# cl-volume-renderer/cl-volume-renderer

Measured on AMD Instinct MI355X. Metric: msamples_per_sec, higher is better.
Workload: dtype f32

## Files before the change

cl_volume_renderer_amd/csrc/bounce_device.hpp:

```cpp
#pragma once
#include "render_device.hpp"

namespace clvr {

__device__ __forceinline__ VolumePacked make_volume(const RenderArgs &a) {
  return VolumePacked{a.grec, a.stepb, a.volume_lin, a.sdf_lin, a.X, a.Y, a.Z, a.NBX, a.NBY};
}

__device__ __forceinline__ uint32_t udivmod24(uint32_t n, uint32_t d, uint32_t &rem) {
  uint32_t q = (uint32_t)((float)n * __builtin_amdgcn_rcpf((float)d));
  uint32_t qd;
  asm("v_mul_u32_u24 %0, %1, %2" : "=v"(qd) : "v"(q), "v"(d));
  int32_t r = (int32_t)(n - qd);
  if (r < 0) { q -= 1u; r += (int32_t)d; }
  if (r >= (int32_t)d) { q += 1u; r -= (int32_t)d; }
  rem = (uint32_t)r;
  return q;
}

__device__ __forceinline__ unsigned prefix_count(unsigned long long mask) {
  return __builtin_amdgcn_mbcnt_hi((unsigned)(mask >> 32), __builtin_amdgcn_mbcnt_lo((unsigned)mask, 0u));
}
__device__ __forceinline__ unsigned lane_id() { return prefix_count(~0ull); }

enum : int { ST_IDLE = 0, ST_MARCH = 1, ST_CERT = 2, ST_EVENT = 8 };
enum : int { EV_START = 3,
             EV_HIT_COLOR_PENDING = 4,
             EV_CHECK = 5 };
constexpr int kCertNever = 255;

template <int MODE>
__device__ __forceinline__ void finish_item(const RenderArgs &a, int64_t entry, uint32_t hit, uint32_t gx, uint32_t gy,
                                            uint32_t bv_r, uint32_t bv_g, uint32_t bv_b) {
  const uint32_t cr = (bv_r / 2u) & 0xFFFFu, cg = (bv_g / 2u) & 0xFFFFu, cb = (bv_b / 2u) & 0xFFFFu;
  if (MODE == CLWH_ACCUM_VOXEL_CACHE && a.grants == nullptr) {
    cache_add(a.cache, entry, cr, cg, cb, 0u);
  } else {
    const unsigned long long packed = (unsigned long long)cr | ((unsigned long long)cg << 16) |
                                      ((unsigned long long)cb << 32) | (1ull << 48);
    atomicAdd(a.delta + hit, packed);
  }
  if (a.contrib_out) {
    uint32_t *q = a.contrib_out + ((size_t)gy * (size_t)a.launch_w + gx) * 4;
    q[0] = cr; q[1] = cg; q[2] = cb; q[3] = 1u;
  }
}

constexpr int kFixupDwords = 32;

__device__ __forceinline__ bool certify_exit(const RenderArgs &a, f3 p, f3 d, int budget, int &away) {
  const unsigned cx = min((unsigned)(int)p.x >> a.macro_shift, (unsigned)a.MNX - 1u), cy = min((unsigned)(int)p.y >> a.macro_shift, (unsigned)a.MNY - 1u),
                 cz = min((unsigned)(int)p.z >> a.macro_shift, (unsigned)a.MNZ - 1u);
  const unsigned octant = (d.x < 0.0f ? 1u : 0u) | (d.y < 0.0f ? 2u : 0u) | (d.z < 0.0f ? 4u : 0u);
  const int entry = a.macro[(((cz * (unsigned)a.MNY + cy) * (unsigned)a.MNX + cx) << 3) | octant];
  const bool refused = (entry & (int)kCertRefused) != 0;
  const int box_min = refused ? 0 : entry;
  away = refused ? ((entry & 0x7F) - 1) << a.macro_shift : 0;
  const float dmin = fminf(fminf(fabsf(d.x), fabsf(d.y)), fabsf(d.z));
  const float dsum = d.x + d.y + d.z;
  const float T = (float)((budget - 5) * box_min);
  const float fx = d.x < 0.0f ? p.x : (float)a.X - p.x, fy = d.y < 0.0f ? p.y : (float)a.Y - p.y, fz = d.z < 0.0f ? p.z : (float)a.Z - p.z;
  const bool leaves = T * fabsf(d.x) >= fx || T * fabsf(d.y) >= fy || T * fabsf(d.z) >= fz;
  return box_min != 0 && budget > 5 && leaves && dmin >= 0.0009765625f && dsum == dsum;
}
__device__ __forceinline__ bool start_certificate(uint32_t mask, f3 d, float dmin_needed) {
  const unsigned octant = (d.x < 0.0f ? 1u : 0u) | (d.y < 0.0f ? 2u : 0u) | (d.z < 0.0f ? 4u : 0u);
  const float dmin = fminf(fminf(fabsf(d.x), fabsf(d.y)), fabsf(d.z));
  const float dsum = d.x + d.y + d.z;
  return ((mask >> octant) & 1u) != 0u && dmin >= dmin_needed && dsum == dsum;
}
__device__ __forceinline__ f3 hull_direction(unsigned k) {
  static_assert(kHullGrid == 64, "cell centres are odd multiples of 1/64");
  const float u = (float)(2 * (int)(k & 63u) - 63) * 0.015625f, v = (float)(2 * (int)((k >> 6) & 63u) - 63) * 0.015625f;
  const float z = (1.0f - fabsf(u)) - fabsf(v);
  const float x = z >= 0.0f ? u : copysignf(1.0f - fabsf(v), u), y = z >= 0.0f ? v : copysignf(1.0f - fabsf(u), v);
  const float r = __builtin_amdgcn_rsqf((x * x + y * y) + z * z);
  return f3{x * r, y * r, z * r};
}
__device__ __forceinline__ bool hull_certificate(uint32_t code, f3 d, float delta0) {
  const f3 n = hull_direction(code - 1u);
  const float dmin = fminf(fminf(fabsf(d.x), fabsf(d.y)), fabsf(d.z));
  const float dsum = d.x + d.y + d.z;
  return code != 0u && dot3(d, n) >= delta0 && dmin >= 0.0009765625f && dsum == dsum;
}
__device__ __forceinline__ bool certify_exit(const RenderArgs &a, f3 p, f3 d, int budget) {
  int away;
  return certify_exit(a, p, d, budget, away);
}

template <int SMALL>
__device__ __forceinline__ void index_tables_to_lds(VolumePacked &vol, const RenderArgs &a, int threads) {
  extern __shared__ uint32_t lds_parts[];
  if (SMALL == 2) {
    vol.parts = lds_parts;
    vol.parts_y0 = a.X;
    vol.parts_z0 = a.X + a.Y;
    for (int k = (int)threadIdx.x; k < a.X + a.Y + a.Z; k += threads)
      lds_parts[k] = k < a.X ? vol.part_x<1>((unsigned)k) : (k < a.X + a.Y ? vol.part_y<1>((unsigned)(k - a.X)) : vol.part_z<1>((unsigned)(k - a.X - a.Y)));
  }
}
__device__ __forceinline__ unsigned home_queue_of(const RenderArgs &a, unsigned waves_per_block) {
  unsigned home_queue = (unsigned)__builtin_amdgcn_s_getreg((3 << 11) | 20) & 7u;
  if (a.unit_affinity == 1) home_queue = (blockIdx.x * waves_per_block + (threadIdx.x >> 6)) & 7u;
  if (a.unit_affinity == 2) home_queue = 0u;
  return home_queue;
}

#ifdef CLVR_BOUNCE_STATS
constexpr bool kBounceStats = true;
constexpr bool kStartCertVerify = (CLVR_BOUNCE_STATS + 0) != 2;
#else
constexpr bool kBounceStats = false;
constexpr bool kStartCertVerify = false;
#endif
template <bool ON> struct BounceStatsT;
template <> struct BounceStatsT<false> {
  __device__ void step(int) {}
  __device__ void cert_begin(int, int) {}
  __device__ void cert_end(int, int) {}
  __device__ void closing_half(int) {}
  __device__ void event_phase(int) {}
  __device__ void refill(uint32_t) {}
  __device__ void fresh_items(int, int) {}
  __device__ void swap_point() {}
  __device__ void start_cert(bool, bool) {}
  __device__ void hull_cert(bool, bool, bool) {}
  __device__ void march_end(uint32_t *, int) {}
  template <bool TWO_RAYS> __device__ void flush(uint32_t *) {}
};
template <> struct BounceStatsT<true> {
  uint32_t step_iters = 0, step_lanes = 0, event_phases = 0, event_lanes = 0, refills = 0, refill_lanes = 0;
  uint32_t ev_kind[4] = {0, 0, 0, 0};
  uint32_t cert_phases = 0, cert_lanes = 0, cert_granted = 0;
  uint32_t step_idle = 0;
  uint32_t swaps = 0;
  uint32_t closing = 0, marching_before = 0;
  __device__ __forceinline__ void step(int st) {
    step_iters += 1; step_lanes += (uint32_t)__popcll(__ballot(st == ST_MARCH));
    step_idle += (uint32_t)__popcll(__ballot(st == ST_IDLE));
  }
  __device__ __forceinline__ void cert_begin(int st, int n_cert) {
    cert_phases += 1; cert_lanes += (uint32_t)n_cert;
    marching_before = (uint32_t)__popcll(__ballot(st == ST_MARCH));
  }
  __device__ __forceinline__ void cert_end(int st, int n_cert) { cert_granted += (uint32_t)(n_cert - (__popcll(__ballot(st == ST_MARCH)) - (int)marching_before)); }
  __device__ __forceinline__ void closing_half(int st) {
    closing = (uint32_t)__popcll(__ballot(st >= ST_EVENT));
    event_lanes += closing;
    ev_kind[1] += (uint32_t)__popcll(__ballot(st == ST_EVENT + EV_EXIT || st == ST_EVENT + EV_CHECK));
    ev_kind[2] += (uint32_t)__popcll(__ballot(st == ST_EVENT + EV_HIT || st == ST_EVENT + EV_HIT_COLOR_PENDING));
    ev_kind[3] += (uint32_t)__popcll(__ballot(st == ST_EVENT + EV_NONE));
  }
  __device__ __forceinline__ void event_phase(int st) {
    if (__ballot(st >= ST_EVENT) != 0ull) { event_phases += 1; event_lanes += (uint32_t)__popcll(__ballot(st >= ST_EVENT)); }
  }
  __device__ __forceinline__ void refill(uint32_t count) { refills += 1; refill_lanes += count; }
  __device__ __forceinline__ void fresh_items(int st, int o) {
    const uint32_t n_fresh = (uint32_t)__popcll(__ballot(st == ST_EVENT + EV_START && o == 1));
    ev_kind[0] += n_fresh; event_lanes += n_fresh;
    if (closing + n_fresh != 0u) event_phases += 1;
  }
  __device__ __forceinline__ void swap_point() { swaps += 1; }
  uint32_t start_tried = 0, start_granted = 0;
  bool start_open = false;
  __device__ __forceinline__ void start_cert(bool tried, bool granted) {
    start_tried += (uint32_t)__popcll(__ballot(tried)); start_granted += (uint32_t)__popcll(__ballot(granted));
    start_open = start_open || granted;
  }
  uint32_t hull_tried = 0, hull_granted = 0, hull_both = 0;
  bool hull_open = false;
  __device__ __forceinline__ void hull_cert(bool tried, bool granted, bool both) {
    hull_tried += (uint32_t)__popcll(__ballot(tried)); hull_granted += (uint32_t)__popcll(__ballot(granted));
    hull_both += (uint32_t)__popcll(__ballot(both));
    hull_open = hull_open || granted;
  }
  __device__ __forceinline__ void march_end(uint32_t *counters, int ev) {
    if (start_open && ev != EV_EXIT) atomicAdd(&counters[CTR_START_WRONG], 1u);
    if (hull_open && ev != EV_EXIT) atomicAdd(&counters[CTR_HULL_WRONG], 1u);
    start_open = false;
    hull_open = false;
  }
  template <bool TWO_RAYS> __device__ __forceinline__ void flush(uint32_t *counters) {
    atomicAdd(&counters[CTR_STEP_ITERS], step_iters); atomicAdd(&counters[CTR_STEP_LANES], step_lanes);
    atomicAdd(&counters[CTR_EVENT_PHASES], event_phases); atomicAdd(&counters[CTR_EVENT_LANES], event_lanes);
    atomicAdd(&counters[CTR_REFILLS], refills); atomicAdd(&counters[CTR_REFILL_LANES], refill_lanes);
    if (TWO_RAYS) { atomicAdd(&counters[CTR_SWAPS], swaps); return; }
    for (int k = 0; k < 4; ++k) atomicAdd(&counters[CTR_EV_KIND + k], ev_kind[k]);
    atomicAdd(&counters[CTR_CERT_PHASES], cert_phases); atomicAdd(&counters[CTR_CERT_LANES], cert_lanes);
    atomicAdd(&counters[CTR_CERT_GRANTED], cert_granted); atomicAdd(&counters[CTR_STEP_IDLE], step_idle);
    atomicAdd(&counters[CTR_START_TRIED], start_tried); atomicAdd(&counters[CTR_START_GRANTED], start_granted);
    atomicAdd(&counters[CTR_HULL_TRIED], hull_tried); atomicAdd(&counters[CTR_HULL_GRANTED], hull_granted); atomicAdd(&counters[CTR_HULL_BOTH], hull_both);
  }
};
using BounceStats = BounceStatsT<kBounceStats>;

}
```

cl_volume_renderer_amd/csrc/clwh_context.hip:

```cpp
#include <algorithm>
#include <cstdio>
#include <cstdlib>
#include <cstring>
#include <mutex>
#include <new>

#include "clwh_host.hpp"

using namespace clvr;

static thread_local int g_last_hip_error = 0;
void clvr::note_hip_error(hipError_t e) { g_last_hip_error = (int)e; }

static std::atomic<uint64_t> g_content_version{0};
static std::mutex g_cells_mutex;
static std::map<const void *, std::weak_ptr<VersionCell>> g_version_cells;
void clwh_touch(clwh_mem *m) { m->cell->v.store(++g_content_version, std::memory_order_relaxed); }

static std::shared_ptr<VersionCell> version_cell_of(const void *dptr) {
  std::lock_guard<std::mutex> lock(g_cells_mutex);
  auto it = g_version_cells.find(dptr);
  if (it != g_version_cells.end())
    if (auto live = it->second.lock()) return live;
  auto cell = std::make_shared<VersionCell>();
  g_version_cells[dptr] = cell;
  if (g_version_cells.size() > 4096) {
    for (auto i = g_version_cells.begin(); i != g_version_cells.end();)
      i = i->second.expired() ? g_version_cells.erase(i) : std::next(i);
  }
  return cell;
}

static size_t elem_size(int kind) {
  switch (kind) {
    case CLWH_ELEM_S8: case CLWH_ELEM_U8: return 1;
    case CLWH_ELEM_S16: case CLWH_ELEM_U16: return 2;
    case CLWH_ELEM_S32: case CLWH_ELEM_U32: case CLWH_ELEM_F32: return 4;
    default: return 0;
  }
}


void clvr::tf_to_dev(const clwh_tf &tf, TfDev &d) {
  std::memset(&d, 0, sizeof d);
  d.n = tf.n;
  for (int k = 0; k < tf.n; ++k) {
    const clwh_tf_rule &r = tf.rules[k];
    TfRuleDev &o = d.rules[k];
    o.v_lo = r.v_lo; o.v_hi = r.v_hi; o.g_lo = r.g_lo; o.g_hi = r.g_hi;
    o.flags = (r.use_gradient ? TF_USE_GRADIENT : 0u) | (r.writes_color ? TF_WRITES_COLOR : 0u) |
              (r.terminal ? TF_TERMINAL : 0u);
    o.color = ((uint32_t)r.color[0] & 255u) | (((uint32_t)r.color[1] & 255u) << 8) |
              (((uint32_t)r.color[2] & 255u) << 16) | (((uint32_t)r.color[3] & 255u) << 24);
    if (r.use_gradient) d.uses_gradient = 1;
  }
  for (int k = 0; k < tf.n && !d.uses_gradient; ++k) {
    const clwh_tf_rule &r = tf.rules[k];
    if (r.v_lo <= 0 && 0 <= r.v_hi) { d.border_class = k + 1; break; }
    if (r.terminal) break;
  }
}

int clvr::jit_for_source(clwh_ctx *ctx, const char *source, std::shared_ptr<JitTf> &out) {
  auto it = ctx->classes.cache.find(source);
  if (it != ctx->classes.cache.end()) {
    out = it->second;
    return CLWH_OK;
  }
  auto j = std::make_shared<JitTf>();
  j->source = source;
  std::string log;
  const int rc = tf_jit_compile(source, j->code, log);
  if (rc != CLWH_OK) {
    if (!log.empty()) std::fprintf(stderr, "clwhip: transfer-function source is neither in the rule grammar nor compilable:\n%s\n", log.c_str());
    return rc;
  }
  ctx->classes.cache[source] = j;
  out = j;
  return CLWH_OK;
}

int clvr::ensure_classes(clwh_ctx *ctx, const std::shared_ptr<JitTf> &jit, const clwh_mem *volume, TfDev &tf_out, const uint8_t **cls_out) {
  TfClasses &c = ctx->classes;
  if (c.cls.ptr && c.vol == volume->dptr && c.vol_ver == volume->version() && c.source == jit->source) {
    tf_out = c.tf;
    *cls_out = c.cls.as<uint8_t>();
    return CLWH_OK;
  }
  if (!jit->module) {
    HIP_TRY(hipModuleLoadData(&jit->module, jit->code.data()));
    HIP_TRY(hipModuleGetFunction(&jit->classify, jit->module, "clvr_tf_classify"));
  }
  const size_t voxels = volume->dims[0] * volume->dims[1] * volume->dims[2];
  CLWH_TRY(c.cls.reserve(ctx->stream, voxels));
  constexpr int kColors = CLWH_TF_MAX_RULES;
  CLWH_TRY(c.palette.reserve(ctx->stream, (kColors + 2) * sizeof(unsigned long long)));
  unsigned long long *palette = c.palette.as<unsigned long long>();
  HIP_TRY(hipMemsetAsync(palette, 0xFF, kColors * sizeof(unsigned long long), ctx->stream));
  HIP_TRY(hipMemsetAsync(palette + kColors, 0, 2 * sizeof(unsigned long long), ctx->stream));
  const void *vol = volume->dptr;
  int X = (int)volume->dims[0], Y = (int)volume->dims[1], Z = (int)volume->dims[2], max_colors = kColors;
  unsigned char *cls = c.cls.as<unsigned char>();
  int *error = reinterpret_cast<int *>(palette + kColors);
  int *border = reinterpret_cast<int *>(palette + kColors + 1);
  void *args[] = {&vol, &X, &Y, &Z, &cls, &palette, &max_colors, &error, &border};
  const size_t blocks = std::min<size_t>((voxels + 255u) / 256u, (size_t)1u << 23);
  HIP_TRY(hipModuleLaunchKernel(jit->classify, (unsigned)blocks, 1, 1, 256, 1, 1, 0, ctx->stream, args, nullptr));
  unsigned long long host[kColors + 2];
  HIP_TRY(hipMemcpyAsync(host, palette, sizeof host, hipMemcpyDeviceToHost, ctx->stream));
  HIP_TRY(hipStreamSynchronize(ctx->stream));
  c.vol = nullptr;
  if ((int)(host[kColors] & 0xFFFFFFFFull) != 0) return CLWH_ERR_TF_UNSUPPORTED;
  TfDev t;
  std::memset(&t, 0, sizeof t);
  t.opaque = 1;
  for (int k = 0; k < kColors && host[k] != ~0ull; ++k) {
    t.rules[k].flags = (host[k] >> 32) & 1ull ? TF_WRITES_COLOR : 0u;
    t.rules[k].color = (uint32_t)(host[k] & 0xFFFFFFFFull);
    t.n = k + 1;
  }
  t.border_class = (int32_t)(host[kColors + 1] & 0xFFull);
  c.tf = t;
  c.vol = volume->dptr;
  c.vol_ver = volume->version();
  c.source = jit->source;
  tf_out = t;
  *cls_out = cls;
  return CLWH_OK;
}


Tuning clvr::tuning_from_environment() {
  Tuning t;
  auto clamped = [](const char *e, int lo, int hi) { return std::max(lo, std::min(hi, std::atoi(e))); };
  if (const char *e = std::getenv("CLWH_TUNE_STEP")) t.step_min_lanes = clamped(e, 0, 64);
  if (const char *e = std::getenv("CLWH_TUNE_REFILL")) t.refill_min_lanes = clamped(e, 0, 64);
  if (const char *e = std::getenv("CLWH_TUNE_LITERAL_GRADIENT")) t.literal_gradient = std::atoi(e) != 0;
  if (const char *e = std::getenv("CLWH_TUNE_AFFINITY")) t.unit_affinity = std::atoi(e);
  if (const char *e = std::getenv("CLWH_TUNE_QUEUES")) t.unit_queues = clamped(e, 1, 8);
  if (const char *e = std::getenv("CLWH_TUNE_GROUP")) t.unit_group = std::max(1, std::atoi(e));
  if (const char *e = std::getenv("CLWH_TUNE_CHUNK_BLOCK_LOG2")) t.unit_block_log2 = clamped(e, 0, 8);
  if (const char *e = std::getenv("CLWH_TUNE_BLOCKS")) t.bounce_max_blocks = (uint32_t)std::max(1, std::atoi(e));
  if (const char *e = std::getenv("CLWH_TUNE_MACRO_SHIFT")) t.macro_shift = std::atoi(e);
  if (const char *e = std::getenv("CLWH_TUNE_LONG_LAUNCH")) t.force_long_launch = std::atoi(e) != 0;
  if (const char *e = std::getenv("CLWH_TUNE_BOUNCE_RAYS")) t.bounce_rays = std::atoi(e) == 2 ? 2 : 1;
  if (const char *e = std::getenv("CLWH_TUNE_SDF")) t.sdf_front = std::strcmp(e, "front") == 0;
  if (const char *e = std::getenv("CLWH_TUNE_DIST_LINES")) t.dist_lines = std::strcmp(e, "scan") == 0 ? 1 : std::strcmp(e, "search") == 0 ? 2 : 0;
  if (const char *e = std::getenv("CLWH_TUNE_LABEL_STATS")) t.label_stats = std::strcmp(e, "item") == 0 ? 1 : std::strcmp(e, "direct") == 0 ? 2 : 0;
  if (const char *e = std::getenv("CLWH_TUNE_SLICE_COARSE")) t.slice_coarse = std::atoi(e) != 0;
  if (const char *e = std::getenv("CLWH_TUNE_SDFBIT_WAVES")) t.sdfbit_waves = std::atoi(e) == 16 ? 16 : 8;
  if (const char *e = std::getenv("CLWH_TUNE_SDFBIT_GRID")) t.sdfbit_grid = std::max(1, std::atoi(e));
  if (const char *e = std::getenv("CLWH_TUNE_SDFBIT_REC")) t.sdfbit_rec_lds = std::strcmp(e, "lds") == 0 ? 1 : 0;
  if (const char *e = std::getenv("CLWH_TUNE_CERT")) t.cert_min_step = clamped(e, 0, 127);
  if (const char *e = std::getenv("CLWH_TUNE_CERT_HINT")) t.cert_hint = std::atoi(e) != 0;
  if (const char *e = std::getenv("CLWH_TUNE_START_CERT")) t.start_cert = std::atoi(e) != 0;
  if (const char *e = std::getenv("CLWH_TUNE_HULL_CERT")) t.hull_cert = std::atoi(e) != 0;
  return t;
}

int clvr::check_device_flags(clwh_ctx *ctx) {
  PassScratch &p = ctx->pass;
  if (!p.fixup_overflow_pending || !p.sticky_flags.ptr) return CLWH_OK;
  uint32_t flag = 0;
  HIP_TRY(hipMemcpyAsync(&flag, p.sticky_flags.ptr, sizeof flag, hipMemcpyDeviceToHost, ctx->stream));
  HIP_TRY(hipStreamSynchronize(ctx->stream));
  p.fixup_overflow_pending = false;
  if (!flag) return CLWH_OK;
  HIP_TRY(hipMemsetAsync(p.sticky_flags.ptr, 0, sizeof(uint32_t), ctx->stream));
  return CLWH_ERR_INTERNAL_OVERFLOW;
}

int clvr::timed_begin(clwh_ctx *ctx, int which, hipEvent_t *end) {
  LaunchTimers &t = ctx->timers;
  if (!t.enabled) return CLWH_OK;
  if (t.used == t.pairs.size()) {
    LaunchTimers::Pair &fresh = t.pairs.emplace_back();
    int rc = fresh.begin.ensure(hipEventDefault);
    if (rc == CLWH_OK) rc = fresh.end.ensure(hipEventDefault);
    if (rc != CLWH_OK) {
      t.pairs.pop_back();
      return rc;
    }
  }
  LaunchTimers::Pair &p = t.pairs[t.used++];
  p.which = which;
  HIP_TRY(hipEventRecord(p.begin.ev, ctx->stream));
  *end = p.end.ev;
  return CLWH_OK;
}

static int order_streams(clwh_ctx *ctx, hipStream_t first, hipStream_t then) {
  HIP_TRY(hipSetDevice(ctx->device));
  CLWH_TRY(ctx->handoff.ensure(hipEventDisableTiming));
  HIP_TRY(hipEventRecord(ctx->handoff.ev, first));
  HIP_TRY(hipStreamWaitEvent(then, ctx->handoff.ev, 0));
  return CLWH_OK;
}

extern "C" {

int clwh_ctx_create_on_stream(int device, void *hip_stream, clwh_ctx **out) {
  if (!out) return CLWH_ERR_INVALID_VALUE;
  *out = nullptr;
  int count = 0;
  hipError_t e = hipGetDeviceCount(&count);
  if (e != hipSuccess || count <= 0) {
    note_hip_error(e);
    return CLWH_ERR_NO_DEVICE;
  }
  if (device < 0 || device >= count) return CLWH_ERR_NO_DEVICE;
  HIP_TRY(hipSetDevice(device));
  clwh_ctx *c = new (std::nothrow) clwh_ctx();
  if (!c) return CLWH_ERR_OUT_OF_MEMORY;
  c->device = device;
  c->stream = (hipStream_t)hip_stream;
  c->own_stream = false;
  c->tune = tuning_from_environment();
  *out = c;
  return CLWH_OK;
}

int clwh_ctx_create(int device, clwh_ctx **out) {
  CLWH_TRY(clwh_ctx_create_on_stream(device, nullptr, out));
  hipStream_t s;
  hipError_t e = hipStreamCreateWithFlags(&s, hipStreamNonBlocking);
  if (e != hipSuccess) {
    note_hip_error(e);
    delete *out;
    *out = nullptr;
    return CLWH_ERR_HIP;
  }
  (*out)->stream = s;
  (*out)->own_stream = true;
  return CLWH_OK;
}

int clwh_ctx_destroy(clwh_ctx *ctx) {
  if (!ctx) return CLWH_ERR_INVALID_VALUE;
  (void)hipSetDevice(ctx->device);
  (void)hipStreamSynchronize(ctx->stream);
  for (auto &kv : ctx->classes.cache)
    if (kv.second->module) (void)hipModuleUnload(kv.second->module);
  ctx->scene.reset();
  const hipStream_t owned = ctx->own_stream ? ctx->stream : nullptr;
  delete ctx;
  if (owned) (void)hipStreamDestroy(owned);
  return CLWH_OK;
}

int clwh_ctx_finish(clwh_ctx *ctx) {
  if (!ctx) return CLWH_ERR_INVALID_VALUE;
  HIP_TRY(hipStreamSynchronize(ctx->stream));
  return check_device_flags(ctx);
}

int clwh_ctx_acquire_from(clwh_ctx *ctx, void *hip_stream) {
  if (!ctx) return CLWH_ERR_INVALID_VALUE;
  return order_streams(ctx, (hipStream_t)hip_stream, ctx->stream);
}

int clwh_ctx_release_to(clwh_ctx *ctx, void *hip_stream) {
  if (!ctx) return CLWH_ERR_INVALID_VALUE;
  return order_streams(ctx, ctx->stream, (hipStream_t)hip_stream);
}

void *clwh_ctx_stream(clwh_ctx *ctx) { return ctx ? (void *)ctx->stream : nullptr; }
int clwh_ctx_device(clwh_ctx *ctx) { return ctx ? ctx->device : -1; }

int clwh_ctx_set_timing(clwh_ctx *ctx, int enabled) {
  if (!ctx) return CLWH_ERR_INVALID_VALUE;
  ctx->timers.enabled = enabled != 0;
  ctx->timers.used = 0;
  return CLWH_OK;
}

int clwh_ctx_timing_read_all(clwh_ctx *ctx, float *ms, int32_t *launches, int32_t n) {
  if (!ctx || !ms || !launches || n <= 0) return CLWH_ERR_INVALID_VALUE;
  for (int k = 0; k < n; ++k) { ms[k] = 0.0f; launches[k] = 0; }
  HIP_TRY(hipSetDevice(ctx->device));
  LaunchTimers &timers = ctx->timers;
  for (size_t i = 0; i < timers.used; ++i) {
    const LaunchTimers::Pair &p = timers.pairs[i];
    HIP_TRY(hipEventSynchronize(p.end.ev));
    float t = 0.0f;
    HIP_TRY(hipEventElapsedTime(&t, p.begin.ev, p.end.ev));
    if (p.which >= 0 && p.which < n) { ms[p.which] += t; launches[p.which] += 1; }
  }
  timers.used = 0;
  return CLWH_OK;
}

int clwh_ctx_timing_read(clwh_ctx *ctx, float *total_ms, int32_t *launches) {
  if (!ctx || !total_ms || !launches) return CLWH_ERR_INVALID_VALUE;
  float ms[CLWH_TIMER_COUNT];
  int32_t n[CLWH_TIMER_COUNT];
  const int rc = clwh_ctx_timing_read_all(ctx, ms, n, CLWH_TIMER_COUNT);
  *total_ms = ms[CLWH_TIMER_BOUNCE];
  *launches = n[CLWH_TIMER_BOUNCE];
  return rc;
}


static int mem_new(clwh_ctx *ctx, void *dptr, size_t bytes, bool owned, clwh_mem **out) {
  clwh_mem *m = new (std::nothrow) clwh_mem();
  if (!m) return CLWH_ERR_OUT_OF_MEMORY;
  m->ctx = ctx;
  m->dptr = dptr;
  m->bytes = bytes;
  m->owned = owned;
// ... 155 lines not shown
```

cl_volume_renderer_amd/csrc/clwh_host.hpp:

```cpp
#pragma once

#include <atomic>
#include <deque>
#include <map>
#include <memory>
#include <string>
#include <vector>

#include "clwh_internal.hpp"

namespace clvr {

void note_hip_error(hipError_t e);
inline int hip_failed(hipError_t e) {
  note_hip_error(e);
  return e == hipErrorOutOfMemory ? CLWH_ERR_OUT_OF_MEMORY : CLWH_ERR_HIP;
}
#define HIP_TRY(expr)                                   \
  do {                                                  \
    hipError_t _e = (expr);                             \
    if (_e != hipSuccess) return clvr::hip_failed(_e);  \
  } while (0)
#define CLWH_TRY(expr)                \
  do {                                \
    int _rc = (expr);                 \
    if (_rc != CLWH_OK) return _rc;   \
  } while (0)

struct NoCopy {
  NoCopy() = default;
  NoCopy(const NoCopy &) = delete;
  NoCopy &operator=(const NoCopy &) = delete;
};

struct DeviceBuffer : NoCopy {
  void *ptr = nullptr;
  size_t bytes = 0;
  ~DeviceBuffer() { if (ptr) (void)hipFree(ptr); }
  template <class T>
  T *as() const { return static_cast<T *>(ptr); }
  void *release() {
    void *p = ptr;
    ptr = nullptr;
    bytes = 0;
    return p;
  }
  int reserve(hipStream_t stream, size_t need, bool *reallocated = nullptr) {
    if (reallocated) *reallocated = bytes < need;
    if (bytes >= need) return CLWH_OK;
    if (ptr) {
      HIP_TRY(hipStreamSynchronize(stream));
      HIP_TRY(hipFree(ptr));
      (void)release();
    }
    HIP_TRY(hipMalloc(&ptr, need));
    bytes = need;
    return CLWH_OK;
  }
};

struct Event : NoCopy {
  hipEvent_t ev = nullptr;
  ~Event() { if (ev) (void)hipEventDestroy(ev); }
  int ensure(unsigned flags) {
    if (!ev) HIP_TRY(hipEventCreateWithFlags(&ev, flags));
    return CLWH_OK;
  }
};

struct PinnedWord : NoCopy {
  uint32_t *ptr = nullptr;
  ~PinnedWord() { if (ptr) (void)hipHostFree(ptr); }
  int ensure() {
    if (!ptr) HIP_TRY(hipHostMalloc((void **)&ptr, 64, hipHostMallocDefault));
    return CLWH_OK;
  }
};

int tf_jit_compile(const char *user_source, std::vector<char> &code, std::string &log);
struct JitTf {
  std::string source;
  std::vector<char> code;
  hipModule_t module = nullptr;
  hipFunction_t classify = nullptr;
};

struct PackedScene {
  int device = 0;
  DeviceBuffer data;
  const void *vol = nullptr, *sdf = nullptr;
  uint64_t vol_ver = 0, sdf_ver = 0;
  TfDev tf{};
  std::string tf_identity;
  int32_t macro_shift = 0;
  bool start_table = false;
  bool hull_table = false;
  int32_t dims[3] = {0, 0, 0};
  uint64_t generation = 0;
  Event ready;
  bool stale = false;
  ~PackedScene();
};

struct VersionCell {
  std::atomic<uint64_t> v{0};
};


struct Tuning {
  int32_t step_min_lanes = 0;
  int32_t refill_min_lanes = 0;
  int32_t macro_shift = 0;
  int32_t bounce_rays = 1;
  int32_t force_long_launch = 0;
  int32_t literal_gradient = 0;
  int32_t unit_block_log2 = 4;
  int32_t unit_group = 1, unit_affinity = 0, unit_queues = 8;
  int32_t cert_hint = 1;
  int32_t start_cert = 1;
  int32_t hull_cert = 1;
  int32_t cert_min_step = -1;
  uint32_t bounce_max_blocks = 2048;
  int32_t sdfbit_waves = 8;
  int32_t sdfbit_grid = 512;
  int32_t sdfbit_rec_lds = 0;
  int32_t sdf_front = 0;
  int32_t dist_lines = 0;
  int32_t label_stats = 0;
  int32_t slice_coarse = 1;
};
Tuning tuning_from_environment();

struct PrimaryHits {
  struct Key {
    float cam_pos[3], cam_dir[3];
    int32_t frame_w, frame_h, launch_w, launch_h, tile_rank, tile_world;
    int64_t cache_entries;
    int32_t mode, shading;
    uint64_t packed_generation;
    const void *env;
    uint64_t env_version;
    int32_t env_w, env_h;
  } key{};
  bool valid = false;
  DeviceBuffer pix_slot, hits;
  DeviceBuffer hull_codes;
  uint32_t n_hits = 0;
  bool n_hits_known = false;
  PinnedWord host_n_hits;
  Event n_hits_event;
  bool n_hits_in_flight = false;
  uint32_t last_known_n_hits = 0;
};

struct PassScratch {
  static constexpr size_t kCounters = CTR_QUEUE_STRIDE * 9;
  DeviceBuffer counters;
  DeviceBuffer fixups, delta;
  DeviceBuffer sticky_flags;
  bool fixup_overflow_pending = false;
};

struct VoxelPlan {
  DeviceBuffer plan;
  DeviceBuffer temp;
  bool valid = false;
  uint32_t n = 0;
};

struct TfClasses {
  std::map<std::string, std::shared_ptr<JitTf>> cache;
  DeviceBuffer cls;
  DeviceBuffer palette;
  const void *vol = nullptr;
  uint64_t vol_ver = 0;
  std::string source;
  TfDev tf{};
};

struct SdfScratch {
  DeviceBuffer counters;
  DeviceBuffer flags;
  DeviceBuffer bits;
#ifdef CLVR_SDFBIT_TIMING
  DeviceBuffer timing;
#endif
};

struct GrowScratch {
  DeviceBuffer admissible, tiles, seeds;
  PinnedWord host;
};

struct LabelScratch {
  DeviceBuffer admissible, keys, temp, counters;
  PinnedWord host;
};

struct DistanceScratch {
  DeviceBuffer map_a, map_b, bits;
};

struct RegionStatsScratch {
  DeviceBuffer result;
};

struct OverlayScratch {
  DeviceBuffer pixel_ids, occupancy;
};

struct ProjectionData {
  DeviceBuffer data;
  bool valid = false;
  const void *vol = nullptr;
  uint64_t vol_ver = 0;
  size_t dims[3] = {0, 0, 0};
  DeviceBuffer dilated;
  bool dilated_valid = false;
  DeviceBuffer mesh_counts, mesh_temp, mesh_points;
  DeviceBuffer lut_prefix;
  bool lut_valid = false;
  const void *lut = nullptr;
  uint64_t lut_ver = 0;
  int32_t lut_len = 0;
};

struct LaunchTimers {
  struct Pair {
    Event begin, end;
    int which = 0;
  };
  bool enabled = false;
  std::deque<Pair> pairs;
  size_t used = 0;
};

}

struct clwh_ctx {
  int device = 0;
  hipStream_t stream = nullptr;
  bool own_stream = false;
  clvr::Event handoff;
  clvr::Tuning tune;
  clvr::PrimaryHits primary;
  clvr::PassScratch pass;
  clvr::VoxelPlan vox;
  clvr::TfClasses classes;
  clvr::SdfScratch sdf;
  clvr::GrowScratch grow;
  clvr::LabelScratch label;
  clvr::DistanceScratch distance;
  clvr::RegionStatsScratch region_stats;
  clvr::OverlayScratch overlay;
  clvr::ProjectionData proj;
  clvr::DeviceBuffer bilateral_weights;
  std::shared_ptr<clvr::PackedScene> scene;
  clvr::LaunchTimers timers;
};

struct clwh_mem {
  clwh_ctx *ctx = nullptr;
  void *dptr = nullptr;
  size_t bytes = 0;
  bool owned = false;
  bool is_image = false;
  size_t dims[3] = {1, 1, 1};
  int channels = 1;
  int elem_kind = CLWH_ELEM_U8;
  int flags = 0;
  std::shared_ptr<clvr::VersionCell> cell;
  uint64_t version() const { return cell ? cell->v.load(std::memory_order_relaxed) : 0; }
};

enum clwh_kernel_id {
  CLWH_K_EMPTY = 0,
  CLWH_K_RENDER,
  CLWH_K_SDF_BASE,
  CLWH_K_SDF_LAYER,
  CLWH_K_BUFFER_RESET,
  CLWH_K_FETCH_STATS,
  CLWH_K_APPLY_CLIP,
  CLWH_K_TF_SORT_VALUES,
  CLWH_K_TF_FLUSH_COLOR_FRAME,
  CLWH_K_BILATERAL_FILTER
};

struct clwh_kernel {
  clwh_ctx *ctx = nullptr;
  int id = CLWH_K_EMPTY;
  clwh_tf tf{};
  bool has_tf = false;
  std::shared_ptr<clvr::JitTf> jit;
};

void clwh_touch(clwh_mem *m);

namespace clvr {

inline void touch(clwh_mem *m) { clwh_touch(m); }

int check_device_flags(clwh_ctx *ctx);

void tf_to_dev(const clwh_tf &tf, TfDev &d);
int jit_for_source(clwh_ctx *ctx, const char *source, std::shared_ptr<JitTf> &out);
int ensure_classes(clwh_ctx *ctx, const std::shared_ptr<JitTf> &jit, const clwh_mem *volume, TfDev &tf_out, const uint8_t **cls_out);
inline int kernel_tf(clwh_kernel *k, const clwh_mem *volume, TfDev &tf_out, const uint8_t **cls_out) {
  if (k->jit) return ensure_classes(k->ctx, k->jit, volume, tf_out, cls_out);
  tf_to_dev(k->tf, tf_out);
// ... 36 lines not shown
```

cl_volume_renderer_amd/csrc/clwh_internal.hpp:

```cpp
#pragma once

#include <hip/hip_runtime.h>
#include <stdint.h>

#include "../../include/clwh.h"

namespace clvr {

struct TfRuleDev {
  int32_t v_lo, v_hi, g_lo, g_hi;
  uint32_t flags;
  uint32_t color;
};
struct TfDev {
  int32_t n;
  int32_t uses_gradient;
  int32_t literal_gradient_taps;
  int32_t opaque;
  int32_t border_class;
  TfRuleDev rules[CLWH_TF_MAX_RULES];
};

enum : uint32_t { TF_USE_GRADIENT = 1u, TF_WRITES_COLOR = 2u, TF_TERMINAL = 4u };

struct HitRec {
  float origin[3];
  float direction[3];
  float normal[3];
  uint32_t color;
  int32_t entry_lo;
  int32_t entry_hi;
  uint32_t xy;
  uint32_t pslot;
  uint32_t start_free;
  uint32_t pad;
};
static_assert(sizeof(HitRec) == 64, "HitRec must be one 64-byte line");

enum : uint32_t { PIX_HIT = 0x80000000u };

constexpr uint32_t kCertMinStep = 2u;
constexpr uint32_t kCertRefused = 0x80u;

enum : uint32_t {
  CTR_HITS = 0, CTR_FIXUPS = 2,
  CTR_STEP_ITERS = 8, CTR_STEP_LANES, CTR_EVENT_PHASES, CTR_EVENT_LANES, CTR_REFILLS, CTR_REFILL_LANES,
  CTR_EV_KIND,
  CTR_CERT_PHASES = CTR_EV_KIND + 4, CTR_CERT_LANES, CTR_CERT_GRANTED,
  CTR_SWAPS, CTR_STEP_IDLE,
  CTR_START_TRIED, CTR_START_GRANTED, CTR_START_WRONG,
  CTR_HULL_TRIED, CTR_HULL_GRANTED, CTR_HULL_BOTH, CTR_HULL_WRONG,
  CTR_STATS_END,
  CTR_QUEUE_STRIDE = 32,
};
struct RenderArgs {
  int32_t X, Y, Z;
  const uint2 *grec;
  const uint8_t *stepb;
  const int16_t *volume_lin;
  const int8_t *sdf_lin;
  const uint8_t *macro;
  int32_t MNX, MNY, MNZ, macro_shift;
  int32_t cert_min_step;
  int32_t cert_min_lanes;
  int32_t cert_hint;
  const uint8_t *start_free;
  float start_cert_dmin;
  const float4 *hull;
  uint32_t *hull_codes;
  float hull_delta0;
  int32_t NBX, NBY;
  const uint32_t *env;
  int32_t env_w, env_h;
  uint32_t *cache;
  int64_t cache_entries;
  uint32_t *frame;
  int32_t frame_w, frame_h;
  int32_t launch_w, launch_h;
  int32_t tiles_x, tiles_y, tiles_per_row;
  int32_t tile_rank, tile_world;
  float cam_pos[3];
  float cam_dir[3];
  int32_t mode;
  float4 *accum;
  unsigned long long *delta;
  const uint32_t *grants;
  uint32_t *pix_slot;
  HitRec *hits;
  uint32_t *counters;
  uint32_t *fixups;
  uint32_t fixup_capacity;
  uint32_t *sticky_flags;
  uint32_t n_hits;
  uint32_t n_hits_estimate;
  int32_t n_hits_on_device;
  int32_t shading;
  int64_t *hit_index_out;
  uint32_t *contrib_out;
  uint32_t num_tile_slots;
  int32_t n_seeds;
  int32_t seeds[CLWH_MAX_SEEDS];
  int32_t step_min_lanes;
  int32_t refill_min_lanes;
  int32_t force_long_launch;
  int32_t bounce_rays;
  uint32_t bounce_max_blocks;
  int32_t unit_group;
  int32_t unit_block_log2;
  int32_t unit_queues;
  int32_t unit_affinity;
  TfDev tf;
};

struct RepackArgs {
  const int16_t *volume;
  const int8_t *sdf;
  int32_t X, Y, Z;
  int32_t NBX, NBY, NBZ;
  uint2 *grec;
  uint8_t *stepb;
  uint32_t *brick_min;
  const uint8_t *cls_in;
  TfDev tf;
};

struct SdfArgs {
  const int16_t *volume;
  int32_t X, Y, Z;
  int8_t *ping;
  int8_t *pong;
  int32_t max_iterations;
  int32_t iteration;
  int32_t *counters;
  int32_t *done;
  int32_t *counter_out;
  const uint8_t *cls_in;
  TfDev tf;
};

hipError_t launch_repack(const RepackArgs &a, hipStream_t s);
inline int macro_cell_shift(int X, int Y, int Z, int forced) {
  if (forced >= 3 && forced <= 8) return forced;
  auto cells = [&](int sh) { return (int64_t)((X >> sh) + 1) * ((Y >> sh) + 1) * ((Z >> sh) + 1); };
  int shift = 4;
  if (cells(4) > 40000) {
    shift = 5;
    while (shift < 8 && cells(shift) > 300000) ++shift;
  }
  return shift;
}
hipError_t launch_macro_table(const uint32_t *brick_min, int NBX, int NBY, int NBZ, uint8_t *macro, int X, int Y, int Z, int shift, hipStream_t s);
hipError_t launch_start_table(const uint8_t *stepb, uint8_t *table, uint32_t *regular, int2 *ends, int X, int Y, int Z, int NBX, int NBY, int NBZ, hipStream_t s);
inline int start_cert_cap(int X, int Y, int Z) {
  const int longest = X > Y ? (X > Z ? X : Z) : (Y > Z ? Y : Z);
  return longest / 2 < 127 ? longest / 2 : 127;
}
inline float start_cert_dmin(int X, int Y, int Z) {
  const double longest = (double)(X > Y ? (X > Z ? X : Z) : (Y > Z ? Y : Z));
  const double reach = 1.7320508075688772 * (longest + 1.0), cap = (double)start_cert_cap(X, Y, Z);
  for (int k = 1; k <= 64; ++k) {
    const double dmin = (double)k / 64.0;
    double t = 0.0;
    for (int step = 0; step < 70 - 5 && t <= reach; ++step) {
      const double m = (double)(long long)(t * dmin) - 2.0;
      const double bound = m > cap ? cap : m;
      t += bound < 1.0 ? 1.0 : bound;
    }
    if (t > reach) return (float)dmin;
  }
  return 2.0f;
}
constexpr int kHullGrid = 64;
constexpr int kHullPlanes = kHullGrid * kHullGrid;
constexpr float kHullSlack = 0.0625f;
constexpr int kHullMaxDim = 2048;
inline float hull_cert_delta0(int X, int Y, int Z) {
  const double longest = (double)(X > Y ? (X > Z ? X : Z) : (Y > Z ? Y : Z));
  const double reach = 1.7320508075688772 * (longest + 1.0), cap = (double)start_cert_cap(X, Y, Z);
  for (int k = 1; k <= 64; ++k) {
    const double delta0 = (double)k / 64.0;
    double t = 0.0;
    for (int step = 0; step < 70 - 5 && t <= reach; ++step) {
      const double m = (double)(long long)(t * delta0 / 1.7320508075688772) - 2.0;
      const double bound = m > cap ? cap : m;
      t += bound < 1.0 ? 1.0 : bound;
    }
    if (t > reach) return (float)delta0;
  }
  return 2.0f;
}
hipError_t launch_hull_table(const int2 *ends, const uint32_t *regular, float4 *hull, int X, int Y, int Z, hipStream_t s);
constexpr uint64_t kStartTableBudget = 2ull << 30;
hipError_t launch_primary(const RenderArgs &a, hipStream_t s);
hipError_t launch_bounce(const RenderArgs &a, hipStream_t s);
inline bool bounce_queues_fit(uint32_t n_hits, int32_t unit_block_log2, int32_t n_seeds) {
  return (uint64_t)(((n_hits + 63u) >> 6) + 8u * (1u << unit_block_log2)) * (uint64_t)n_seeds < (1ull << 24);
}
hipError_t launch_env_fixup(const RenderArgs &a, hipStream_t s);
hipError_t launch_commit(const RenderArgs &a, hipStream_t s);
constexpr int64_t kVoxKeyInvalid = (int64_t)1 << 38;
constexpr int64_t kVoxKeyNone = ((int64_t)1 << 38) + 1;
hipError_t launch_vox_keys(const RenderArgs &a, int64_t *keys, uint32_t *iota, uint32_t n, hipStream_t s);
hipError_t launch_vox_grant(const RenderArgs &a, const int64_t *sorted_keys, const uint32_t *order, uint32_t n, uint32_t *grants, hipStream_t s);
hipError_t launch_commit_voxel(const RenderArgs &a, hipStream_t s);
hipError_t sort_entry_pairs(void *temp, size_t &temp_bytes, const int64_t *keys_in, int64_t *keys_out, const uint32_t *vals_in,
                            uint32_t *vals_out, size_t n, unsigned end_bit, hipStream_t s);
hipError_t launch_resolve(const RenderArgs &a, hipStream_t s);
hipError_t launch_ao(const RenderArgs &a, hipStream_t s);
hipError_t launch_accum_resolve(const RenderArgs &a, const float4 *accum_all, hipStream_t s);
hipError_t launch_accum_resolve_tiles(const RenderArgs &a, const float4 *accum, uint32_t *tiles_out, hipStream_t s);
hipError_t launch_frame_from_tiles(const RenderArgs &a, const uint32_t *tiles_all, hipStream_t s);
struct SdfFrontArgs {
  int8_t *sdf;
  int32_t X, Y, Z;
  int32_t TX, TY, TZ;
  const uint8_t *flags_cur;
  uint8_t *flags_next;
  uint8_t *flags_clear;
  uint8_t *tile_done;
  int32_t iteration;
  int32_t max_iterations;
  int32_t *counters;
};

struct SdfBitArgs {
  int8_t *sdf;
  const uint32_t *ev;
  const uint32_t *r_in;
  uint32_t *r_out;
  uint8_t *state;
  uint8_t *wake;
  int32_t launch;
  int32_t *presence;
  int32_t X, Y, Z, WP;
  int32_t BX, BY, BZ, core_z;
  int32_t r0, steps;
  uint32_t *planes;
  size_t plane_words;
  uint32_t *list;
  uint32_t *list_count;
  uint32_t *list_head;
#ifdef CLVR_SDFBIT_TIMING
  unsigned long long *timing;
#endif
};
void sdfbit_block_grid(int X, int Y, int Z, int waves, int32_t *BX, int32_t *BY, int32_t *BZ, int32_t *core_z);
hipError_t launch_sdfbit_events(const SdfArgs &a, uint32_t *ev, int32_t WP, hipStream_t s);
hipError_t launch_sdfbit_seed(const SdfBitArgs &a, hipStream_t s);
hipError_t launch_sdfbit_expand(const SdfBitArgs &a, const uint32_t *reached, int32_t max_iterations, hipStream_t s);
hipError_t launch_sdfbit_state(const SdfBitArgs &a, hipStream_t s);
hipError_t launch_sdfbit_layers(const SdfBitArgs &a, int waves, unsigned grid_blocks, bool rec_in_lds, hipStream_t s);

inline unsigned row_block(int X) { return X <= 64 ? 64u : (X <= 128 ? 128u : 256u); }
inline dim3 row_grid(int X, int Y, int Z) { return dim3(((unsigned)X + row_block(X) - 1u) / row_block(X), (unsigned)Y, (unsigned)Z); }
hipError_t launch_sdf_base(const SdfArgs &a, hipStream_t s);
hipError_t launch_sdf_base_front(const SdfArgs &a, uint8_t *flags, int32_t TX, int32_t TY, hipStream_t s);
hipError_t launch_sdf_front(const SdfFrontArgs &a, hipStream_t s);
hipError_t launch_sdf_layer(const SdfArgs &a, hipStream_t s);
hipError_t launch_fetch_stats(const int16_t *vol, int X, int Y, int Z, int32_t *stats, hipStream_t s);
hipError_t launch_tf_sort_values(const int16_t *vol, int X, int Y, int Z, uint32_t *frame, int width, int height,
                                 float min_v, float max_v, float min_g, float max_g, hipStream_t s);
hipError_t launch_tf_flush_color_frame(uint32_t *color_frame, int fw, int fh, const int32_t *frame, const int32_t *lookup,
                                       int lookup_len, hipStream_t s);
hipError_t launch_bilateral_filter(const int16_t *src, int X, int Y, int Z, int16_t *dst, const float *weights, hipStream_t s);
hipError_t launch_apply_clip(const int16_t *src, int SX, int SY, int SZ, int16_t *dst, int DX, int DY, int DZ,
                             const uint32_t *start, const uint32_t *len, hipStream_t s);


struct ViewVolume {
  const int16_t *bricks;
  const uint32_t *table, *dilated, *coarse;
  int32_t X, Y, Z, NBX, NBY, NBZ, CNX, CNY;
};
struct ViewFrame {
  uint32_t *frame;
  int32_t frame_w, frame_h;
  int32_t launch_w, launch_h, tiles_x, num_tiles;
};
struct ViewCamera {
  float cam_pos[3], cam_dir[3];
  float step, t_near, t_far;
  int32_t k_cap;
};

struct ProjRepackArgs {
  const int16_t *volume;
  int32_t X, Y, Z, NBX, NBY, NBZ;
  int16_t *bricks;
  uint32_t *table;
};
struct ProjArgs {
  ViewVolume vol;
  ViewFrame fr;
  ViewCamera cam;
  float window_center, window_width;
  float *values;
  float *t_extreme;
};
hipError_t launch_proj_repack(const ProjRepackArgs &a, hipStream_t s);
hipError_t launch_projection(const ProjArgs &a, int mode, bool dense, hipStream_t s);

struct CompArgs {
  ViewVolume vol;
  ViewFrame fr;
  ViewCamera cam;
  const float4 *lut;
  const uint32_t *prefix;
  int32_t lut_first, lut_len;
  float alpha_stop, ambient;
  float4 *rgba;
  float *t_first;
  float *t_stop;
};
hipError_t launch_comp_prefix(const float4 *lut, int32_t lut_len, uint32_t *prefix, hipStream_t s);
hipError_t launch_composite(const CompArgs &a, bool shade, bool dense, hipStream_t s);

struct IsoArgs {
  ViewVolume vol;
  ViewFrame fr;
  ViewCamera cam;
  int64_t threshold;
  int32_t skip_bound;
  int32_t refine;
  float color[3], ambient;
  float *t_hit;
  float4 *normal;
};
hipError_t launch_iso_dilate(const ViewVolume &v, uint32_t *dilated, hipStream_t s);
hipError_t launch_isosurface(const IsoArgs &a, bool below, bool dense, hipStream_t s);

struct SliceArgs {
  ViewVolume vol;
  ViewFrame fr;
  int32_t use_coarse;
  float origin[3], du[3], dv[3], normal[3];
  float step;
  float window_center, window_width;
  int32_t slab_samples;
  float *values;
  float *t_extreme;
};
hipError_t launch_slice(const SliceArgs &a, int mode, bool dense, hipStream_t s);

// ... 136 lines not shown
```

cl_volume_renderer_amd/csrc/clwh_render.hip:

```cpp
#include <algorithm>
#include <cstdio>
#include <cstring>
#include <mutex>

#include "clwh_host.hpp"

using namespace clvr;


static std::mutex g_scenes_mutex;
static std::vector<std::weak_ptr<PackedScene>> g_packed_scenes;
static std::atomic<uint64_t> g_packed_generation{0};

PackedScene::~PackedScene() {
  (void)hipSetDevice(device);
  (void)hipDeviceSynchronize();
}

struct PackedLayout {
  int X, Y, Z, NBX, NBY, NBZ, mshift, MNX, MNY, MNZ;
  size_t records, n_bricks, off_stepb, off_brick_min, off_macro, off_start, off_hull_ends, off_hull, bytes;
  bool start_table;
  bool hull_table;
};
// ... 60 lines not shown
    entry = std::make_shared<PackedScene>();
    entry->device = ctx->device;
    CLWH_TRY(entry->data.reserve(ctx->stream, L.bytes));
    CLWH_TRY(entry->ready.ensure(hipEventDisableTiming));
  }
  ctx->scene.reset();
  {
    std::lock_guard<std::mutex> lock(g_scenes_mutex);
    entry->stale = true;
  }
  uint8_t *data = entry->data.as<uint8_t>();
  RepackArgs r;
  std::memset(&r, 0, sizeof r);
  r.volume = (const int16_t *)volume->dptr;
  r.sdf = (const int8_t *)sdf->dptr;
  r.X = L.X; r.Y = L.Y; r.Z = L.Z;
  r.NBX = L.NBX; r.NBY = L.NBY; r.NBZ = L.NBZ;
  r.grec = reinterpret_cast<uint2 *>(data);
  r.stepb = data + L.off_stepb;
  r.brick_min = reinterpret_cast<uint32_t *>(data + L.off_brick_min);
  HIP_TRY(hipMemsetAsync(r.brick_min, 0xFF, L.n_bricks * sizeof(uint32_t), ctx->stream));
  r.cls_in = cls_in;
  r.tf = tf;
  CLWH_TRY(timed(ctx, CLWH_TIMER_REPACK, [&] {
    const hipError_t e = launch_repack(r, ctx->stream);
    if (e != hipSuccess) return e;
    return launch_macro_table(r.brick_min, L.NBX, L.NBY, L.NBZ, data + L.off_macro, L.X, L.Y, L.Z, L.mshift, ctx->stream);
  }));
  if (L.start_table)
    CLWH_TRY(timed(ctx, CLWH_TIMER_REPACK, [&] {
      int2 *ends = L.hull_table ? reinterpret_cast<int2 *>(data + L.off_hull_ends) : nullptr;
      const hipError_t e = launch_start_table(r.stepb, data + L.off_start + 16u, reinterpret_cast<uint32_t *>(data + L.off_start), ends, L.X, L.Y, L.Z, L.NBX, L.NBY, L.NBZ, ctx->stream);
      if (e != hipSuccess || !L.hull_table) return e;
      return launch_hull_table(ends, reinterpret_cast<const uint32_t *>(data + L.off_start), reinterpret_cast<float4 *>(data + L.off_hull), L.X, L.Y, L.Z, ctx->stream);
    }));
  HIP_TRY(hipEventRecord(entry->ready.ev, ctx->stream));
  ctx->scene = entry;
  {
    std::lock_guard<std::mutex> lock(g_scenes_mutex);
    entry->vol = volume->dptr;
    entry->sdf = sdf->dptr;
    entry->vol_ver = volume->version();
    entry->sdf_ver = sdf->version();
    entry->tf = tf;
    entry->tf_identity = tf_identity;
    entry->macro_shift = L.mshift;
    entry->start_table = L.start_table;
    entry->hull_table = L.hull_table;
    entry->dims[0] = L.X; entry->dims[1] = L.Y; entry->dims[2] = L.Z;
    entry->generation = ++g_packed_generation;
    entry->stale = false;
    bool listed = false;
    for (auto &w : g_packed_scenes)
      if (w.lock() == entry) listed = true;
    if (!listed) g_packed_scenes.push_back(entry);
  }
  return CLWH_OK;
}


static void describe_frame(RenderArgs &a, int32_t launch_w, int32_t launch_h, int32_t frame_w, int32_t frame_h,
                           int32_t rank, int32_t world, const float cam_pos[3], const float cam_dir[3]) {
  a.launch_w = launch_w;
  a.launch_h = launch_h;
  a.frame_w = frame_w;
  a.frame_h = frame_h;
  a.tiles_x = launch_w / 8;
  a.tiles_y = launch_h / 8;
  a.tile_rank = rank;
  a.tile_world = world;
  a.tiles_per_row = (a.tiles_x + world - 1) / world;
  a.num_tile_slots = (uint32_t)a.tiles_y * (uint32_t)a.tiles_per_row;
  for (int q = 0; q < 3; ++q) {
    a.cam_pos[q] = cam_pos[q];
    a.cam_dir[q] = cam_dir[q];
  }
}

static size_t pixel_slots(const RenderArgs &a) { return (size_t)a.num_tile_slots * 64u; }
static size_t launch_pixels(const RenderArgs &a) { return (size_t)a.launch_w * (size_t)a.launch_h; }
static bool is_planned(const RenderArgs &a) { return a.mode == CLWH_ACCUM_VOXEL_CACHE && a.n_seeds > 1; }

static int validate_desc(const clwh_render_desc *d) {
  if (!is_image(d->volume, 3, 1, CLWH_ELEM_S16) || !is_image(d->sdf, 3, 1, CLWH_ELEM_S8) ||
      !is_image(d->env, 2, 4, CLWH_ELEM_U8))
    return CLWH_ERR_BAD_ARGS;
  if (d->frame && !is_image(d->frame, 2, 4, CLWH_ELEM_U8)) return CLWH_ERR_BAD_ARGS;
  if (!same_dims(d->volume, d->sdf)) return CLWH_ERR_SIZE_MISMATCH;
  if (!launch_size_ok(d->width, d->height)) return CLWH_ERR_BAD_NDRANGE;
  if (d->width > 65535u || d->height > 65535u) return CLWH_ERR_BAD_NDRANGE;
  if (d->env->dims[0] > 32768u || d->env->dims[1] > 32768u) return CLWH_ERR_INVALID_VALUE;
  if (!dims_fit_int32(d->volume)) return CLWH_ERR_INVALID_VALUE;
  const int world = d->tile_world < 1 ? 1 : d->tile_world;
  if (d->tile_rank < 0 || d->tile_rank >= world) return CLWH_ERR_INVALID_VALUE;
  if (d->n_seeds < 0 || d->n_seeds > CLWH_MAX_SEEDS) return CLWH_ERR_INVALID_VALUE;
  if (d->n_seeds > 1 && d->contrib) return CLWH_ERR_BAD_ARGS;
  if (d->shading != CLWH_SHADE_LIGHT && d->shading != CLWH_SHADE_AO) return CLWH_ERR_INVALID_VALUE;
  if (d->shading == CLWH_SHADE_AO && d->accum_mode != CLWH_ACCUM_VOXEL_CACHE) return CLWH_ERR_BAD_ARGS;
  return CLWH_OK;
}

static int describe_launch(const clwh_ctx *ctx, const clwh_render_desc *d, RenderArgs &a) {
  std::memset(&a, 0, sizeof a);
  a.X = (int32_t)d->volume->dims[0];
  a.Y = (int32_t)d->volume->dims[1];
  a.Z = (int32_t)d->volume->dims[2];
  env_into_args(a, d->env);
  const int32_t fw = d->frame ? (int32_t)d->frame->dims[0] : (int32_t)d->width;
  const int32_t fh = d->frame ? (int32_t)d->frame->dims[1] : (int32_t)d->height;
  const int world = d->tile_world < 1 ? 1 : d->tile_world;
  describe_frame(a, (int32_t)d->width, (int32_t)d->height, fw, fh, d->tile_rank, world, d->cam_pos, d->cam_dir);
  a.frame = d->frame ? (uint32_t *)d->frame->dptr : nullptr;
  a.mode = d->accum_mode;
  a.shading = d->shading;
  if (a.mode == CLWH_ACCUM_VOXEL_CACHE) {
    if (!d->buffer_volume || d->buffer_volume->bytes < 8) return CLWH_ERR_BAD_ARGS;
    a.cache = (uint32_t *)d->buffer_volume->dptr;
    a.cache_entries = (int64_t)(d->buffer_volume->bytes / (d->shading == CLWH_SHADE_AO ? 4 : 8));
  } else if (a.mode == CLWH_ACCUM_IMAGE_SPACE) {
    const int64_t need = clwh_accum_len(d->width, d->height, world) * 16;
    if (!d->accum || (int64_t)d->accum->bytes < need) return CLWH_ERR_BAD_ARGS;
    a.accum = (float4 *)d->accum->dptr;
  } else {
    return CLWH_ERR_INVALID_VALUE;
  }
  if (d->hit_index) {
    if (d->hit_index->bytes < launch_pixels(a) * 8) return CLWH_ERR_SIZE_MISMATCH;
    a.hit_index_out = (int64_t *)d->hit_index->dptr;
  }
  if (d->contrib) {
    if (d->contrib->bytes < launch_pixels(a) * 16) return CLWH_ERR_SIZE_MISMATCH;
    a.contrib_out = (uint32_t *)d->contrib->dptr;
  }
  if (d->n_seeds > 0) {
    a.n_seeds = d->n_seeds;
    for (int q = 0; q < d->n_seeds; ++q) a.seeds[q] = d->seeds[q];
  } else {
    a.n_seeds = 1;
    a.seeds[0] = d->seed;
  }
  const Tuning &t = ctx->tune;
  a.step_min_lanes = t.step_min_lanes;
  a.refill_min_lanes = t.refill_min_lanes;
  a.force_long_launch = t.force_long_launch;
  a.bounce_rays = t.bounce_rays;
  a.bounce_max_blocks = t.bounce_max_blocks;
  a.unit_group = t.unit_group;
  a.unit_block_log2 = t.unit_block_log2;
  a.unit_affinity = t.unit_affinity;
  a.unit_queues = t.unit_queues;
  a.cert_hint = t.cert_hint;
  a.start_cert_dmin = start_cert_dmin(a.X, a.Y, a.Z);
  a.hull_delta0 = hull_cert_delta0(a.X, a.Y, a.Z);
  return CLWH_OK;
}

static int bind_scene(clwh_kernel *k, const clwh_render_desc *d, RenderArgs &a) {
  clwh_ctx *ctx = k->ctx;
  const uint8_t *cls_in = nullptr;
  CLWH_TRY(kernel_tf(k, d->volume, a.tf, &cls_in));
  a.tf.literal_gradient_taps = ctx->tune.literal_gradient;
  const PackedLayout L = packed_layout(d->volume, ctx->tune.macro_shift, wants_start_table(ctx->tune, a.tf, d->volume), wants_hull_table(ctx->tune, a.tf, d->volume));
  CLWH_TRY(ensure_packed(ctx, L, d->volume, d->sdf, a.tf, cls_in, k->jit ? k->jit->source : std::string()));
  const uint8_t *packed = ctx->scene->data.as<uint8_t>();
  a.grec = reinterpret_cast<const uint2 *>(packed);
  a.NBX = L.NBX;
  a.NBY = L.NBY;
  a.stepb = packed + L.off_stepb;
  a.volume_lin = (const int16_t *)d->volume->dptr;
  a.sdf_lin = (const int8_t *)d->sdf->dptr;
  a.macro = packed + L.off_macro;
  a.start_free = L.start_table ? packed + L.off_start + 16u : nullptr;
  a.hull = L.hull_table ? reinterpret_cast<const float4 *>(packed + L.off_hull) : nullptr;
  a.macro_shift = L.mshift;
  a.MNX = L.MNX; a.MNY = L.MNY; a.MNZ = L.MNZ;
  bool zero_may_hit = a.tf.border_class != 0;
  for (int q = 0; q < a.tf.n && a.tf.uses_gradient && !a.tf.opaque; ++q)
    if (a.tf.rules[q].v_lo <= 0 && 0 <= a.tf.rules[q].v_hi) zero_may_hit = true;
  const int cert_auto = a.macro_shift < 4 ? 12 >> (4 - a.macro_shift) : std::min(12 << (a.macro_shift - 4), 48);
  a.cert_min_step = zero_may_hit ? 0 : (ctx->tune.cert_min_step >= 0 ? ctx->tune.cert_min_step : cert_auto);
  return CLWH_OK;
}

static int ensure_primary_hits(clwh_ctx *ctx, const clwh_render_desc *d, RenderArgs &a) {
  PrimaryHits &p = ctx->primary;
  PassScratch &s = ctx->pass;
  const size_t slots = pixel_slots(a);
  CLWH_TRY(p.pix_slot.reserve(ctx->stream, slots * sizeof(uint32_t)));
  CLWH_TRY(p.hits.reserve(ctx->stream, slots * sizeof(HitRec)));
  if (a.hull) CLWH_TRY(p.hull_codes.reserve(ctx->stream, slots * sizeof(uint32_t)));
  CLWH_TRY(s.counters.reserve(ctx->stream, PassScratch::kCounters * sizeof(uint32_t)));
  bool fresh_flags = false;
  CLWH_TRY(s.sticky_flags.reserve(ctx->stream, 64, &fresh_flags));
  if (fresh_flags) HIP_TRY(hipMemsetAsync(s.sticky_flags.ptr, 0, 64, ctx->stream));
  a.sticky_flags = s.sticky_flags.as<uint32_t>();
  a.pix_slot = p.pix_slot.as<uint32_t>();
  a.hits = p.hits.as<HitRec>();
  a.hull_codes = a.hull ? p.hull_codes.as<uint32_t>() : nullptr;
  a.counters = s.counters.as<uint32_t>();

  PrimaryHits::Key key;
  std::memset(&key, 0, sizeof key);
  for (int q = 0; q < 3; ++q) {
    key.cam_pos[q] = a.cam_pos[q];
    key.cam_dir[q] = a.cam_dir[q];
  }
  key.frame_w = a.frame_w; key.frame_h = a.frame_h;
  key.launch_w = a.launch_w; key.launch_h = a.launch_h;
  key.tile_rank = a.tile_rank; key.tile_world = a.tile_world;
  key.cache_entries = a.cache_entries;
  key.mode = a.mode;
  key.shading = a.shading;
  key.packed_generation = ctx->scene->generation;
  key.env = d->env->dptr;
  key.env_version = d->env->version();
  key.env_w = a.env_w; key.env_h = a.env_h;
  if (p.valid && std::memcmp(&key, &p.key, sizeof key) == 0 && !a.hit_index_out) return CLWH_OK;
  p.valid = false;
  HIP_TRY(hipMemsetAsync(a.counters, 0, PassScratch::kCounters * sizeof(uint32_t), ctx->stream));
  CLWH_TRY(timed(ctx, CLWH_TIMER_PRIMARY, [&] { return launch_primary(a, ctx->stream); }));
  CLWH_TRY(p.host_n_hits.ensure());
  CLWH_TRY(p.n_hits_event.ensure(hipEventDisableTiming));
  HIP_TRY(hipMemcpyAsync(p.host_n_hits.ptr, a.counters + CTR_HITS, sizeof(uint32_t), hipMemcpyDeviceToHost, ctx->stream));
  HIP_TRY(hipEventRecord(p.n_hits_event.ev, ctx->stream));
  p.n_hits_in_flight = true;
  ctx->vox.valid = false;
  p.n_hits_known = false;
  p.key = key;
  p.valid = true;
  return CLWH_OK;
}

static int pick_up_hit_count(clwh_ctx *ctx, RenderArgs &a) {
  PrimaryHits &p = ctx->primary;
  if (p.n_hits_in_flight && !p.n_hits_known) {
    if (hipEventQuery(p.n_hits_event.ev) == hipSuccess) {
      p.n_hits = *p.host_n_hits.ptr;
      p.n_hits_known = true;
      p.n_hits_in_flight = false;
      p.last_known_n_hits = p.n_hits;
    } else {
      (void)hipGetLastError();
    }
  }
  const size_t slots = pixel_slots(a);
  a.n_hits_on_device = !p.n_hits_known;
  a.n_hits = p.n_hits_known ? p.n_hits : (uint32_t)std::min<size_t>(slots, 0xFFFFFFFFu);
  a.n_hits_estimate = a.n_hits;
  if (!p.n_hits_known && p.last_known_n_hits != 0)
    a.n_hits_estimate = (uint32_t)std::min<uint64_t>(a.n_hits, std::max<uint64_t>(2ull * p.last_known_n_hits, slots / 4u));
  if (!bounce_queues_fit(a.n_hits, ctx->tune.unit_block_log2, a.n_seeds)) return CLWH_ERR_INVALID_VALUE;
  return CLWH_OK;
}

static int size_pass_buffers(clwh_ctx *ctx, RenderArgs &a) {
  PassScratch &s = ctx->pass;
  const double rate = std::min(1.0, std::max(1.0 / 64.0, 3.0 * 8.0e-6 * (0.16 * a.env_w + 0.32 * a.env_h)));
  const size_t fix_cap = std::max<size_t>((size_t)((double)a.n_hits_estimate * (double)a.n_seeds * rate), 4096u);
  CLWH_TRY(s.fixups.reserve(ctx->stream, fix_cap * 128u));
  a.fixups = s.fixups.as<uint32_t>();
  a.fixup_capacity = (uint32_t)std::min<size_t>(s.fixups.bytes / 128u, 0x7fffffffu);
  if (a.mode == CLWH_ACCUM_IMAGE_SPACE || is_planned(a)) {
    bool fresh = false;
    CLWH_TRY(s.delta.reserve(ctx->stream, std::max<size_t>(pixel_slots(a), 1) * sizeof(unsigned long long), &fresh));
    a.delta = s.delta.as<unsigned long long>();
    if (fresh) HIP_TRY(hipMemsetAsync(s.delta.ptr, 0, s.delta.bytes, ctx->stream));
  }
  return CLWH_OK;
}

static int plan_voxel_grants(clwh_ctx *ctx, RenderArgs &a) {
  if (!is_planned(a)) return CLWH_OK;
  VoxelPlan &v = ctx->vox;
  constexpr size_t kPerElement = 2 * sizeof(int64_t) + 3 * sizeof(uint32_t);
  bool moved = false;
  CLWH_TRY(v.plan.reserve(ctx->stream, pixel_slots(a) * kPerElement, &moved));
  if (moved) v.valid = false;
  const size_t have = v.plan.bytes / kPerElement;
  int64_t *keys_in = v.plan.as<int64_t>(), *keys = keys_in + have;
  uint32_t *iota = reinterpret_cast<uint32_t *>(keys + have), *order = iota + have, *grants = order + have;
  if (!v.valid) {
    const uint32_t n = a.n_hits;
    HIP_TRY(launch_vox_keys(a, keys_in, iota, n, ctx->stream));
    size_t need = 0;
    HIP_TRY(sort_entry_pairs(nullptr, need, keys_in, keys, iota, order, n, 39u, ctx->stream));
    CLWH_TRY(v.temp.reserve(ctx->stream, std::max<size_t>(need, 16)));
    size_t tb = v.temp.bytes;
    HIP_TRY(sort_entry_pairs(v.temp.ptr, tb, keys_in, keys, iota, order, n, 39u, ctx->stream));
    v.valid = true;
    v.n = n;
  }
  HIP_TRY(launch_vox_grant(a, keys, order, v.n, grants, ctx->stream));
  a.grants = grants;
  return CLWH_OK;
}

#ifdef CLVR_BOUNCE_STATS
static int print_bounce_stats(clwh_ctx *ctx, const RenderArgs &a) {
  uint32_t h[CTR_STATS_END];
  HIP_TRY(hipMemcpyAsync(h, a.counters, sizeof h, hipMemcpyDeviceToHost, ctx->stream));
  HIP_TRY(hipStreamSynchronize(ctx->stream));
  auto per = [&](int sum, int n) { return h[n] ? (double)h[sum] / h[n] : 0.0; };
  std::fprintf(stderr, "[bounce stats] items=%llu step_iters=%u avg_march_lanes=%.2f event_phases=%u avg_event_lanes=%.2f "
               "refills=%u avg_refill=%.2f events start/exit/hit/none=%u/%u/%u/%u cert_phases=%u avg_cert_lanes=%.2f cert_granted=%u\n",
               (unsigned long long)h[CTR_HITS] * (unsigned long long)a.n_seeds, h[CTR_STEP_ITERS], per(CTR_STEP_LANES, CTR_STEP_ITERS),
               h[CTR_EVENT_PHASES], per(CTR_EVENT_LANES, CTR_EVENT_PHASES), h[CTR_REFILLS], per(CTR_REFILL_LANES, CTR_REFILLS), h[CTR_EV_KIND],
               h[CTR_EV_KIND + 1], h[CTR_EV_KIND + 2], h[CTR_EV_KIND + 3], h[CTR_CERT_PHASES], per(CTR_CERT_LANES, CTR_CERT_PHASES), h[CTR_CERT_GRANTED]);
  if (h[CTR_SWAPS]) std::fprintf(stderr, "[bounce stats] two rays per lane: %u swap points\n", h[CTR_SWAPS]);
  std::fprintf(stderr, "[bounce stats] per step iteration: avg_idle_lanes=%.2f (lane sum %u)\n", per(CTR_STEP_IDLE, CTR_STEP_ITERS), h[CTR_STEP_IDLE]);
  std::fprintf(stderr, "[bounce stats] lane_steps=%u event_lanes=%u start certificates (%s) tried/granted/wrong=%u/%u/%u dmin=%.6f\n", h[CTR_STEP_LANES],
               h[CTR_EVENT_LANES], (CLVR_BOUNCE_STATS + 0) == 2 ? "taken" : "verified: marched literally", h[CTR_START_TRIED], h[CTR_START_GRANTED],
               h[CTR_START_WRONG], (double)a.start_cert_dmin);
  std::fprintf(stderr, "[bounce stats] hull certificates tried/granted/wrong=%u/%u/%u, of the granted the octant proof grants %u; either proof grants %u first legs; delta0=%.6f\n",
               h[CTR_HULL_TRIED], h[CTR_HULL_GRANTED], h[CTR_HULL_WRONG], h[CTR_HULL_BOTH], h[CTR_START_GRANTED] + h[CTR_HULL_GRANTED] - h[CTR_HULL_BOTH],
               (double)a.hull_delta0);
  return CLWH_OK;
}
#endif

static int run_pass(clwh_ctx *ctx, const RenderArgs &a) {
  CLWH_TRY(timed(ctx, CLWH_TIMER_BOUNCE, [&] { return launch_bounce(a, ctx->stream); }));
#ifdef CLVR_BOUNCE_STATS
  CLWH_TRY(print_bounce_stats(ctx, a));
#endif
  CLWH_TRY(timed(ctx, CLWH_TIMER_FIXUP, [&] {
    hipError_t e = launch_env_fixup(a, ctx->stream);
    if (e == hipSuccess) e = launch_commit(a, ctx->stream);
    if (e == hipSuccess && is_planned(a)) e = launch_commit_voxel(a, ctx->stream);
    return e;
  }));
  ctx->pass.fixup_overflow_pending = true;
  return CLWH_OK;
}

extern "C" {

int64_t clwh_cache_len(uint32_t X, uint32_t Y, uint32_t Z) {
  return ((int64_t)X * Z * Y + (int64_t)X * Z + X + 1) * 4;
}

int64_t clwh_accum_len(uint32_t width, uint32_t height, int32_t tile_world) {
  if (tile_world < 1) tile_world = 1;
  const int64_t tiles_x = width / 8, tiles_y = height / 8;
  const int64_t tiles_per_row = (tiles_x + tile_world - 1) / tile_world;
  return tiles_y * tiles_per_row * 64;
}

int clwh_render(clwh_kernel *k, const clwh_render_desc *d) {
  if (!k || !d || k->id != CLWH_K_RENDER || !k->has_tf) return CLWH_ERR_INVALID_VALUE;
  clwh_ctx *ctx = k->ctx;
  RenderArgs a;
  CLWH_TRY(validate_desc(d));
  CLWH_TRY(describe_launch(ctx, d, a));
  HIP_TRY(hipSetDevice(ctx->device));
  CLWH_TRY(bind_scene(k, d, a));
  CLWH_TRY(ensure_primary_hits(ctx, d, a));
  CLWH_TRY(pick_up_hit_count(ctx, a));

  HIP_TRY(hipMemsetAsync(a.counters + CTR_HITS + 1, 0, (PassScratch::kCounters - CTR_HITS - 1) * sizeof(uint32_t), ctx->stream));
  if (a.contrib_out) HIP_TRY(hipMemsetAsync(a.contrib_out, 0, launch_pixels(a) * 16, ctx->stream));

  if (d->resolve_only) {
    if (!a.frame) return CLWH_ERR_BAD_ARGS;
  } else if (d->shading == CLWH_SHADE_AO) {
    CLWH_TRY(timed(ctx, CLWH_TIMER_AO, [&] { return launch_ao(a, ctx->stream); }));
  } else {
    CLWH_TRY(size_pass_buffers(ctx, a));
    CLWH_TRY(plan_voxel_grants(ctx, a));
    CLWH_TRY(run_pass(ctx, a));
  }
  if ((d->write_frame || d->resolve_only) && a.frame)
    CLWH_TRY(timed(ctx, CLWH_TIMER_RESOLVE, [&] { return launch_resolve(a, ctx->stream); }));
  if (d->frame) touch(d->frame);
  return CLWH_OK;
}


int clwh_accum_resolve(clwh_ctx *ctx, clwh_mem *accum_all, int32_t tile_world, uint32_t width, uint32_t height,
                       clwh_mem *frame, clwh_mem *env, const float cam_pos[3], const float cam_dir[3]) {
  if (!ctx || !accum_all || !frame || !env || !cam_pos || !cam_dir || tile_world < 1) return CLWH_ERR_INVALID_VALUE;
  if (!is_image(frame, 2, 4, CLWH_ELEM_U8) || !is_image(env, 2, 4, CLWH_ELEM_U8)) return CLWH_ERR_BAD_ARGS;
  if (!launch_size_ok(width, height)) return CLWH_ERR_BAD_NDRANGE;
  const int64_t need = clwh_accum_len(width, height, tile_world) * 16 * tile_world;
  if ((int64_t)accum_all->bytes < need) return CLWH_ERR_SIZE_MISMATCH;
  RenderArgs a;
  std::memset(&a, 0, sizeof a);
  describe_frame(a, (int32_t)width, (int32_t)height, (int32_t)frame->dims[0], (int32_t)frame->dims[1], 0, tile_world,
                 cam_pos, cam_dir);
  a.frame = (uint32_t *)frame->dptr;
  env_into_args(a, env);
  HIP_TRY(hipSetDevice(ctx->device));
  CLWH_TRY(timed(ctx, CLWH_TIMER_RESOLVE, [&] { return launch_accum_resolve(a, (const float4 *)accum_all->dptr, ctx->stream); }));
  touch(frame);
  return CLWH_OK;
}

int clwh_accum_resolve_tiles(clwh_ctx *ctx, clwh_mem *accum, int32_t tile_rank, int32_t tile_world, uint32_t width, uint32_t height,
                             clwh_mem *tiles_rgba8, clwh_mem *env, const float cam_pos[3], const float cam_dir[3]) {
  if (!ctx || !accum || !tiles_rgba8 || !env || !cam_pos || !cam_dir || tile_world < 1 || tile_rank < 0 || tile_rank >= tile_world)
    return CLWH_ERR_INVALID_VALUE;
  if (!is_image(env, 2, 4, CLWH_ELEM_U8)) return CLWH_ERR_BAD_ARGS;
  if (!launch_size_ok(width, height)) return CLWH_ERR_BAD_NDRANGE;
  const int64_t n = clwh_accum_len(width, height, tile_world);
  if ((int64_t)accum->bytes < n * 16 || (int64_t)tiles_rgba8->bytes < n * 4) return CLWH_ERR_SIZE_MISMATCH;
  RenderArgs a;
  std::memset(&a, 0, sizeof a);
  describe_frame(a, (int32_t)width, (int32_t)height, (int32_t)width, (int32_t)height, tile_rank, tile_world, cam_pos, cam_dir);
  env_into_args(a, env);
  HIP_TRY(hipSetDevice(ctx->device));
  CLWH_TRY(timed(ctx, CLWH_TIMER_RESOLVE, [&] {
    return launch_accum_resolve_tiles(a, (const float4 *)accum->dptr, (uint32_t *)tiles_rgba8->dptr, ctx->stream);
  }));
  touch(tiles_rgba8);
  return CLWH_OK;
}

int clwh_frame_from_tiles(clwh_ctx *ctx, clwh_mem *tiles_all, int32_t tile_world, uint32_t width, uint32_t height, clwh_mem *frame) {
  if (!ctx || !tiles_all || !frame || tile_world < 1) return CLWH_ERR_INVALID_VALUE;
  if (!is_image(frame, 2, 4, CLWH_ELEM_U8)) return CLWH_ERR_BAD_ARGS;
  if (!launch_size_ok(width, height)) return CLWH_ERR_BAD_NDRANGE;
  if ((int64_t)tiles_all->bytes < clwh_accum_len(width, height, tile_world) * 4 * tile_world) return CLWH_ERR_SIZE_MISMATCH;
  const float zero[3] = {0.0f, 0.0f, 0.0f};
  RenderArgs a;
  std::memset(&a, 0, sizeof a);
  describe_frame(a, (int32_t)width, (int32_t)height, (int32_t)frame->dims[0], (int32_t)frame->dims[1], 0, tile_world, zero, zero);
  a.frame = (uint32_t *)frame->dptr;
  HIP_TRY(hipSetDevice(ctx->device));
  HIP_TRY(launch_frame_from_tiles(a, (const uint32_t *)tiles_all->dptr, ctx->stream));
  touch(frame);
  return CLWH_OK;
}


int clwh_ctx_invalidate_derived(clwh_ctx *ctx, int what) {
  if (!ctx) return CLWH_ERR_INVALID_VALUE;
  if ((what & CLWH_DERIVED_SCENE) && ctx->scene) {
    {
      std::lock_guard<std::mutex> lock(g_scenes_mutex);
      ctx->scene->stale = true;
    }
    if (ctx->scene.use_count() > 1) ctx->scene.reset();
  }
  if (what & (CLWH_DERIVED_SCENE | CLWH_DERIVED_CAMERA)) ctx->primary.valid = false;
  if (what & CLWH_DERIVED_PROJECTION) ctx->proj.valid = ctx->proj.lut_valid = ctx->proj.dilated_valid = false;
  return CLWH_OK;
}

int clwh_ctx_scene_info(clwh_ctx *ctx, uint64_t *scene_id, uint64_t *bytes, int32_t *holders) {
  if (!ctx) return CLWH_ERR_INVALID_VALUE;
  std::lock_guard<std::mutex> lock(g_scenes_mutex);
  if (scene_id) *scene_id = ctx->scene ? ctx->scene->generation : 0;
  if (bytes) *bytes = ctx->scene ? ctx->scene->data.bytes : 0;
  if (holders) *holders = ctx->scene ? (int32_t)ctx->scene.use_count() : 0;
  return CLWH_OK;
}

static PackedLayout scene_layout(clwh_ctx *ctx) {
  std::lock_guard<std::mutex> lock(g_scenes_mutex);
  clwh_mem shape{};
  for (int q = 0; q < 3; ++q) shape.dims[q] = (size_t)ctx->scene->dims[q];
  return packed_layout(&shape, ctx->scene->macro_shift, ctx->scene->start_table, ctx->scene->hull_table);
}

int clwh_debug_macro_table(clwh_ctx *ctx, void *host_out, uint64_t capacity, int32_t info_out[4]) {
  if (!ctx || !info_out) return CLWH_ERR_INVALID_VALUE;
  if (!ctx->scene) return CLWH_ERR_BAD_ARGS;
  const PackedLayout L = scene_layout(ctx);
  info_out[0] = L.MNX; info_out[1] = L.MNY; info_out[2] = L.MNZ; info_out[3] = L.mshift;
  const size_t bytes = (size_t)L.MNX * L.MNY * L.MNZ * 8u;
  if (!host_out) return CLWH_OK;
  if (capacity < bytes || ctx->scene->data.bytes != L.bytes) return CLWH_ERR_SIZE_MISMATCH;
  HIP_TRY(hipSetDevice(ctx->device));
  HIP_TRY(hipMemcpyAsync(host_out, ctx->scene->data.as<uint8_t>() + L.off_macro, bytes, hipMemcpyDeviceToHost, ctx->stream));
  HIP_TRY(hipStreamSynchronize(ctx->stream));
  return CLWH_OK;
}

int clwh_debug_start_table(clwh_ctx *ctx, void *host_out, uint64_t capacity, int32_t info_out[4]) {
  if (!ctx || !info_out) return CLWH_ERR_INVALID_VALUE;
  if (!ctx->scene) return CLWH_ERR_BAD_ARGS;
  const PackedLayout L = scene_layout(ctx);
  info_out[0] = L.X; info_out[1] = L.Y; info_out[2] = L.Z; info_out[3] = L.start_table ? 1 : 0;
  if (!host_out || !L.start_table) return CLWH_OK;
  const size_t bytes = (size_t)L.X * L.Y * L.Z;
  if (capacity < bytes || ctx->scene->data.bytes != L.bytes) return CLWH_ERR_SIZE_MISMATCH;
  HIP_TRY(hipSetDevice(ctx->device));
  HIP_TRY(hipMemcpyAsync(host_out, ctx->scene->data.as<uint8_t>() + L.off_start + 16u, bytes, hipMemcpyDeviceToHost, ctx->stream));
  HIP_TRY(hipStreamSynchronize(ctx->stream));
  return CLWH_OK;
}

int clwh_debug_start_cert_dmin(int32_t X, int32_t Y, int32_t Z, float *dmin_out) {
  if (!dmin_out || X < 1 || Y < 1 || Z < 1) return CLWH_ERR_INVALID_VALUE;
  *dmin_out = start_cert_dmin(X, Y, Z);
  return CLWH_OK;
}

int clwh_debug_hull_table(clwh_ctx *ctx, void *host_out, uint64_t capacity, int32_t info_out[4]) {
  if (!ctx || !info_out) return CLWH_ERR_INVALID_VALUE;
  if (!ctx->scene) return CLWH_ERR_BAD_ARGS;
  const PackedLayout L = scene_layout(ctx);
  info_out[0] = kHullGrid; info_out[1] = kHullPlanes; info_out[2] = 0; info_out[3] = L.hull_table ? 1 : 0;
  if (!host_out || !L.hull_table) return CLWH_OK;
  const size_t bytes = (size_t)kHullPlanes * sizeof(float4);
  if (capacity < bytes || ctx->scene->data.bytes != L.bytes) return CLWH_ERR_SIZE_MISMATCH;
  HIP_TRY(hipSetDevice(ctx->device));
  HIP_TRY(hipMemcpyAsync(host_out, ctx->scene->data.as<uint8_t>() + L.off_hull, bytes, hipMemcpyDeviceToHost, ctx->stream));
  HIP_TRY(hipStreamSynchronize(ctx->stream));
  return CLWH_OK;
}

int clwh_debug_hull_cert_bound(int32_t X, int32_t Y, int32_t Z, float out[2]) {
  if (!out || X < 1 || Y < 1 || Z < 1) return CLWH_ERR_INVALID_VALUE;
  out[0] = hull_cert_delta0(X, Y, Z);
  out[1] = kHullSlack;
  return CLWH_OK;
}

int clwh_debug_hull_codes(clwh_ctx *ctx, void *host_out, uint64_t capacity, uint32_t *n_hits_out) {
  if (!ctx || !n_hits_out) return CLWH_ERR_INVALID_VALUE;
  PrimaryHits &p = ctx->primary;
  if (!p.valid || !p.hits.ptr || !ctx->pass.counters.ptr) return CLWH_ERR_BAD_ARGS;
  HIP_TRY(hipSetDevice(ctx->device));
  HIP_TRY(hipMemcpyAsync(n_hits_out, ctx->pass.counters.as<uint32_t>() + CTR_HITS, sizeof(uint32_t), hipMemcpyDeviceToHost, ctx->stream));
  HIP_TRY(hipStreamSynchronize(ctx->stream));
  if (!host_out) return CLWH_OK;
  const bool built = ctx->scene && ctx->scene->hull_table && p.hull_codes.ptr;
  const size_t bytes = (size_t)*n_hits_out * sizeof(uint32_t);
  if (capacity < bytes || (built && p.hull_codes.bytes < bytes)) return CLWH_ERR_SIZE_MISMATCH;
  if (!built) { std::memset(host_out, 0, bytes); return CLWH_OK; }
  HIP_TRY(hipMemcpyAsync(host_out, p.hull_codes.ptr, bytes, hipMemcpyDeviceToHost, ctx->stream));
  HIP_TRY(hipStreamSynchronize(ctx->stream));
  return CLWH_OK;
}

int clwh_debug_hit_records(clwh_ctx *ctx, void *host_out, uint64_t capacity, uint32_t *n_hits_out) {
  if (!ctx || !n_hits_out) return CLWH_ERR_INVALID_VALUE;
  PrimaryHits &p = ctx->primary;
  if (!p.valid || !p.hits.ptr || !ctx->pass.counters.ptr) return CLWH_ERR_BAD_ARGS;
  HIP_TRY(hipSetDevice(ctx->device));
  HIP_TRY(hipMemcpyAsync(n_hits_out, ctx->pass.counters.as<uint32_t>() + CTR_HITS, sizeof(uint32_t), hipMemcpyDeviceToHost, ctx->stream));
  HIP_TRY(hipStreamSynchronize(ctx->stream));
  if (!host_out) return CLWH_OK;
  const size_t bytes = (size_t)*n_hits_out * sizeof(HitRec);
  if (capacity < bytes || p.hits.bytes < bytes) return CLWH_ERR_SIZE_MISMATCH;
  HIP_TRY(hipMemcpyAsync(host_out, p.hits.ptr, bytes, hipMemcpyDeviceToHost, ctx->stream));
  HIP_TRY(hipStreamSynchronize(ctx->stream));
  return CLWH_OK;
}

}
```

cl_volume_renderer_amd/csrc/primary_kernels.hip:

```cpp
#include "bounce_device.hpp"

namespace clvr {

template <bool USE_GRAD>
__global__ __launch_bounds__(64) void k_primary(const RenderArgs a) {
  const uint32_t slot = xcd_contiguous_slot(blockIdx.x, a.num_tile_slots);
  int tx, ty;
  if (!tile_from_slot(a, slot, tx, ty)) return;
  const uint32_t lane = threadIdx.x;
  const uint32_t x = (uint32_t)tx * 8u + (lane & 7u);
  const uint32_t y = (uint32_t)ty * 8u + (lane >> 3);
  const uint32_t pslot = slot * 64u + lane;

  const VolumePacked vol = make_volume(a);
  const f3 cam_o = f3{a.cam_pos[0], a.cam_pos[1], a.cam_pos[2]};
  const f3 cam_d = f3{a.cam_dir[0], a.cam_dir[1], a.cam_dir[2]};
  const Ray vray = generate_ray(cam_o, cam_d, (int)x, (int)y, a.frame_w, a.frame_h);
  const float dx = (float)a.X, dy = (float)a.Y, dz = (float)a.Z;

  bool cut_ok;
  f3 cut_point;
  if (!(within(vray.origin.x, dx) && within(vray.origin.y, dy) && within(vray.origin.z, dz))) {
    cut_ok = cut_box(dx, dy, dz, vray, cut_point);
  } else {
    cut_ok = true;
    cut_point = vray.origin;
  }

  bool hit = false;
  Ray current_ray{cut_point, vray.direction};
  uint32_t current_color = 0u;
  if (cut_ok) {
    int ev;
    current_ray = march_to_next_event<USE_GRAD>(vol, a.tf, current_ray, ev, current_color);
    hit = (ev == EV_HIT);
  }

  const unsigned long long hit_mask = __ballot(hit);
  uint32_t base = 0u;
  if (hit_mask != 0ull) {
    const int leader = __ffsll((long long)hit_mask) - 1;
    if ((int)lane == leader) base = atomicAdd(&a.counters[CTR_HITS], (uint32_t)__popcll(hit_mask));
    base = __shfl(base, leader);
  }

  constexpr int kHullCoarse = kHullGrid / 4;
  __shared__ float4 hull_coarse[kHullCoarse * kHullCoarse];
  if (a.hull != nullptr && hit_mask != 0ull) {
    for (int c = (int)lane; c < kHullCoarse * kHullCoarse; c += 64)
      hull_coarse[c] = a.hull[((c / kHullCoarse) * 4 + 2) * kHullGrid + (c % kHullCoarse) * 4 + 2];
    __syncthreads();
  }

  int64_t raw_entry = -1;
  if (hit) {
    const uint32_t h = base + prefix_count(hit_mask);
    const f3 normal = -normalize3(gradient_nn(vol, current_ray.origin));
    raw_entry = cache_entry_of(a.X, a.Z, current_ray.origin);
    int64_t entry = raw_entry;
    if (a.mode == CLWH_ACCUM_VOXEL_CACHE && !(entry >= 0 && entry < a.cache_entries)) entry = -2;
    uint4 q0, q1, q2, q3;
    q0.x = __float_as_uint(current_ray.origin.x); q0.y = __float_as_uint(current_ray.origin.y);
    q0.z = __float_as_uint(current_ray.origin.z); q0.w = __float_as_uint(current_ray.direction.x);
    q1.x = __float_as_uint(current_ray.direction.y); q1.y = __float_as_uint(current_ray.direction.z);
    q1.z = __float_as_uint(normal.x); q1.w = __float_as_uint(normal.y);
    q2.x = __float_as_uint(normal.z); q2.y = current_color;
    q2.z = (uint32_t)((uint64_t)entry & 0xFFFFFFFFull); q2.w = (uint32_t)((uint64_t)entry >> 32);
    uint32_t start_free = 0u;
    if (a.start_free) {
      const f3 p = (current_ray.origin + current_ray.direction) + normal * 2.0f;
      if (__float_as_uint(p.x) < __float_as_uint(dx) && __float_as_uint(p.y) < __float_as_uint(dy) && __float_as_uint(p.z) < __float_as_uint(dz))
        start_free = a.start_free[((size_t)(int)p.z * (size_t)a.Y + (size_t)(int)p.y) * (size_t)a.X + (size_t)(int)p.x];
    }
    if (a.hull) {
      const f3 p = (current_ray.origin + current_ray.direction) + normal * 2.0f;
      float best = -INFINITY;
      int bc = 0;
#pragma unroll 4
      for (int c = 0; c < kHullCoarse * kHullCoarse; ++c) {
        const float4 e = hull_coarse[c];
        const float m = ((e.x * p.x + e.y * p.y) + e.z * p.z) - e.w;
        if (m > best) { best = m; bc = c; }
      }
      int bi = (bc % kHullCoarse) * 4 + 2, bj = (bc / kHullCoarse) * 4 + 2;
      uint32_t code = 0u;
      float margin = best;
      const int i0 = bi, j0 = bj;
#pragma unroll 1
      for (int dj = -3; dj <= 3; ++dj)
        for (int di = -3; di <= 3; ++di) {
          const int i = min(max(i0 + di, 0), kHullGrid - 1), j = min(max(j0 + dj, 0), kHullGrid - 1);
          const float4 e = a.hull[j * kHullGrid + i];
          const float m = ((e.x * p.x + e.y * p.y) + e.z * p.z) - e.w;
          if (m >= margin) { margin = m; bi = i; bj = j; }
        }
      if (margin >= 0.0f) code = ((uint32_t)(bj * kHullGrid + bi) + 1u) | ((uint32_t)fminf(floorf(margin * 256.0f), 65535.0f) << 16);
      a.hull_codes[h] = code;
    }
    q3.x = x | (y << 16); q3.y = pslot; q3.z = start_free; q3.w = 0u;
    uint4 *dst = reinterpret_cast<uint4 *>(&a.hits[h]);
    dst[0] = q0; dst[1] = q1; dst[2] = q2; dst[3] = q3;
    a.pix_slot[pslot] = PIX_HIT | h;
  } else {
    const uint32_t e = sample_environment_map(a.env, a.env_w, a.env_h, vray.direction);
    a.pix_slot[pslot] = e & 0x00FFFFFFu;
  }
  if (a.hit_index_out) a.hit_index_out[(size_t)y * (size_t)a.launch_w + x] = raw_entry;
}

template <bool USE_GRAD>
__global__ __launch_bounds__(256) void k_ao(const RenderArgs a) {
  const uint32_t n_hits = a.n_hits_on_device ? a.counters[CTR_HITS] : a.n_hits;
  const uint32_t h = blockIdx.x * blockDim.x + threadIdx.x;
  if (h >= n_hits) return;
  const VolumePacked vol = make_volume(a);
  const uint4 *src = reinterpret_cast<const uint4 *>(&a.hits[h]);
  const uint4 q0 = src[0], q1 = src[1], q2 = src[2], q3 = src[3];
  const f3 hit_origin = f3{__uint_as_float(q0.x), __uint_as_float(q0.y), __uint_as_float(q0.z)};
  const f3 hit_direction = f3{__uint_as_float(q0.w), __uint_as_float(q1.x), __uint_as_float(q1.y)};
  const f3 normal = f3{__uint_as_float(q1.z), __uint_as_float(q1.w), __uint_as_float(q2.x)};
  const int64_t entry = (int64_t)(((uint64_t)q2.w << 32) | (uint64_t)q2.z);
  const uint32_t gx = q3.x & 0xFFFFu, gy = q3.x >> 16;
  if (entry < 0) return;
  uint32_t *word = a.cache + entry;
  for (int s = 0; s < a.n_seeds; ++s) {
    const uint32_t old = atomicAdd(word, 1u);
    uint32_t granted = 1u, occluded = 0u;
    if ((old & 0xFFFFu) >= 100u) {
      atomicSub(word, 1u);
      granted = 0u;
    } else {
      Ray r{hit_origin + hit_direction, hemisphere_direction(gx, gy, normal, a.seeds[s])};
      for (int k = 0; k < 7; ++k) {
        const int sd = (int)(vol.step_i(f2i(r.origin.x), f2i(r.origin.y), f2i(r.origin.z)) & 0x7Fu);
        r.origin = r.origin + r.direction * cl_max((float)sd, 0.5f);
      }
      int ev;
      uint32_t color = 0u;
      march_to_next_event<USE_GRAD>(vol, a.tf, r, ev, color);
      if (ev == EV_HIT) {
        atomicAdd(word, 0x10000u);
        occluded = 1u;
      }
    }
    if (a.contrib_out) {
      uint32_t *q = a.contrib_out + ((size_t)gy * (size_t)a.launch_w + gx) * 4;
      q[0] = occluded; q[1] = 0u; q[2] = 0u; q[3] = granted;
    }
  }
}

hipError_t launch_primary(const RenderArgs &a, hipStream_t s) {
  if (a.tf.uses_gradient)
    hipLaunchKernelGGL(k_primary<true>, dim3(a.num_tile_slots), dim3(64), 0, s, a);
  else
    hipLaunchKernelGGL(k_primary<false>, dim3(a.num_tile_slots), dim3(64), 0, s, a);
  return hipGetLastError();
}
hipError_t launch_ao(const RenderArgs &a, hipStream_t s) {
  if (a.n_hits == 0) return hipSuccess;
  const dim3 grid((a.n_hits + 255u) / 256u), block(256);
  if (a.tf.uses_gradient) hipLaunchKernelGGL(k_ao<true>, grid, block, 0, s, a);
  else hipLaunchKernelGGL(k_ao<false>, grid, block, 0, s, a);
  return hipGetLastError();
}

}
```

cl_volume_renderer_amd/csrc/render_kernels.hip:

```cpp
#include <algorithm>

#include "bounce_two_rays.hpp"

namespace clvr {

#ifndef CLVR_CERT_PHASE_MIN_LANES
#define CLVR_CERT_PHASE_MIN_LANES 16
#endif
constexpr int kCertPhaseMinLanes = CLVR_CERT_PHASE_MIN_LANES;
#ifndef CLVR_BOUNCE_WAVES_PER_SIMD
#define CLVR_BOUNCE_WAVES_PER_SIMD 7
#endif
#ifndef CLVR_BOUNCE_THREADS
#define CLVR_BOUNCE_THREADS 256
#endif
constexpr int kBounceThreads = CLVR_BOUNCE_THREADS;

template <bool USE_GRAD, int MODE, bool SMALL_VOLUME>
__global__ __launch_bounds__(kBounceThreads, CLVR_BOUNCE_WAVES_PER_SIMD) void k_bounce(const RenderArgs a) {
  constexpr int SMALL = SMALL_VOLUME ? 2 : 0;
  VolumePacked vol = make_volume(a);
  index_tables_to_lds<SMALL>(vol, a, kBounceThreads);
  __shared__ float div255[256];
  if (threadIdx.x < 256u) div255[threadIdx.x] = (float)threadIdx.x / 255.0f;
  __syncthreads();
  const uint32_t n_hits = a.n_hits_on_device ? a.counters[CTR_HITS] : a.n_hits;
  const uint32_t n_chunks = (n_hits + 63u) >> 6;
  const unsigned lane = lane_id();
  const unsigned home_queue = home_queue_of(a, (unsigned)(kBounceThreads / 64));
  unsigned queue_dry = 0u;
  enum : int { C_START_X, C_START_Y, C_START_Z,
               C_NORMAL_X, C_NORMAL_Y, C_NORMAL_Z,
               C_ENTRY_LO,
               C_ENTRY_HI,
               C_PIXEL, C_HIT, C_SEED,
               C_FIX,
               C_BV_R, C_BV_G, C_BV_B, C_FIELDS };
  __shared__ uint32_t cold[C_FIELDS][kBounceThreads];
#define COLD(f) cold[f][threadIdx.x]
#define COLD_ENTRY_HI() ((uint32_t)((int32_t)(COLD(C_ENTRY_HI) << 24) >> 24))
  Ray ray{{0, 0, 0}, {0, 0, 0}};
  float atten = 0.0f, r_energy = 0.0f, g_energy = 0.0f, b_energy = 0.0f;
  uint32_t color = 0u;
  int o = 0, i = 0;
  int st = ST_IDLE;
  int sd = 0;
  uint32_t march = 0u;
  constexpr uint32_t kOneStep = 1u << 24, kCertReady = 1u << 23;
  const bool cert_hint = a.cert_hint != 0;
  const int cert_min_lanes = a.cert_min_lanes;
  const int cert_at = a.cert_min_step != 0 ? a.cert_min_step : kCertNever;
  const bool start_cert = !USE_GRAD && a.cert_min_step != 0;
  const bool hull_cert = start_cert && a.hull_codes != nullptr;
  bool exhausted = false;
  BounceStats stats;

  for (;;) {
    if (__ballot(st == ST_MARCH) != 0ull) {
      do {
        stats.step(st);
        if (st == ST_MARCH) {
          ray.origin = ray.origin + ray.direction * fmaxf((float)sd, 0.5f);
          march += (uint32_t)sd - kOneStep;
          if (!USE_GRAD) {
            const bool has_voxel = __float_as_uint(ray.origin.x) < __float_as_uint((float)a.X) &&
                                   __float_as_uint(ray.origin.y) < __float_as_uint((float)a.Y) &&
                                   __float_as_uint(ray.origin.z) < __float_as_uint((float)a.Z);
            if (has_voxel) {
              const unsigned q = vol.template step_marched<SMALL>(ray.origin.x, ray.origin.y, ray.origin.z);
              sd = (int)(q & 0x7Fu);
              if (q & 0x80u) st = ST_EVENT + EV_HIT_COLOR_PENDING;
              else if (march < kOneStep) st = ST_EVENT + EV_NONE;
              else if (sd >= cert_at && (march & kCertReady)) st = ST_CERT;
            } else {
              st = ST_EVENT + EV_CHECK;
            }
          } else if (exited_volume(vol, ray.origin)) {
            st = ST_EVENT + EV_EXIT;
          } else {
            int next_sd;
            bool pending = false;
            const bool is_hit = classify_step<USE_GRAD, SMALL, true>(vol, a.tf, ray.origin, color, next_sd, &pending);
            if (is_hit) {
              st = ST_EVENT + (pending ? EV_HIT_COLOR_PENDING : EV_HIT);
            } else if (march < kOneStep) {
              st = ST_EVENT + EV_NONE;
            } else {
              sd = next_sd;
              if (sd >= cert_at && (march & kCertReady)) st = ST_CERT;
            }
          }
        }
        const int n_cert = __popcll(__ballot(st == ST_CERT));
        if (n_cert != 0 && (n_cert >= cert_min_lanes || __popcll(__ballot(st == ST_MARCH)) < a.step_min_lanes)) {
          stats.cert_begin(st, n_cert);
          if (st == ST_CERT) {
            int away;
            if (certify_exit(a, ray.origin, ray.direction, (int)(march >> 24), away)) {
              st = ST_EVENT + EV_EXIT;
            } else {
              march = (march & ~(kOneStep - 1u)) | (kCertReady - (uint32_t)(cert_hint ? away : 0));
              st = ST_MARCH;
            }
          }
          stats.cert_end(st, n_cert);
        }
      } while (__popcll(__ballot(st == ST_MARCH)) >= a.step_min_lanes);
    }

    stats.closing_half(st);
    if (st >= ST_EVENT) {
      int ev = st - ST_EVENT;
      if (ev == EV_CHECK) {
        for (;;) {
          if (exited_volume(vol, ray.origin)) { ev = EV_EXIT; break; }
          int next_sd;
          bool pending = false;
          if (classify_step<USE_GRAD, SMALL, true>(vol, a.tf, ray.origin, color, next_sd, &pending)) {
            ev = pending ? EV_HIT_COLOR_PENDING : EV_HIT;
            break;
          }
          if (march < kOneStep) { ev = EV_NONE; break; }
          ray.origin = ray.origin + ray.direction * fmaxf((float)next_sd, 0.5f);
          march -= kOneStep;
        }
      }
      stats.march_end(a.counters, ev);
      bool ended = false;

      if (ev == EV_EXIT) {
        const float factor = i == 8 ? 8.0f / 8.0f : (i == 9 ? 8.0f / 9.0f : (i == 10 ? 8.0f / 10.0f : 8.0f / (float)i));
        const float p_r = atten * r_energy, p_g = atten * g_energy, p_b = atten * b_energy;
        uint32_t light = 0u;
        const uint32_t fix_word = COLD(C_FIX);
        int fix = (int)(fix_word >> 2) - 2, npend = (int)(fix_word & 3u);
        bool certain = (fix == -1) && sample_environment_map_fast(a.env, a.env_w, a.env_h, ray.direction, light);
        if (certain) {
          COLD(C_BV_R) = f2u((float)COLD(C_BV_R) + p_r * (float)(light & 255u) * factor / 1.0f);
          COLD(C_BV_G) = f2u((float)COLD(C_BV_G) + p_g * (float)((light >> 8) & 255u) * factor / 1.0f);
          COLD(C_BV_B) = f2u((float)COLD(C_BV_B) + p_b * (float)((light >> 16) & 255u) * factor / 1.0f);
        } else {
          if (fix == -1) {
            const uint32_t slot = atomicAdd(&a.counters[CTR_FIXUPS], 1u);
            if (slot < a.fixup_capacity) {
              fix = (int)slot;
              uint32_t *rec = a.fixups + (size_t)slot * kFixupDwords;
              rec[0] = COLD(C_HIT);
              rec[1] = COLD(C_ENTRY_LO);
              rec[2] = COLD_ENTRY_HI();
              rec[3] = COLD(C_PIXEL);
              rec[4] = COLD(C_BV_R); rec[5] = COLD(C_BV_G); rec[6] = COLD(C_BV_B);
            } else {
              a.sticky_flags[0] = 1u;
              fix = -2;
            }
          }
          if (fix >= 0) {
            uint32_t *e = a.fixups + (size_t)fix * kFixupDwords + 8 + 7 * npend;
            e[0] = __float_as_uint(p_r); e[1] = __float_as_uint(p_g); e[2] = __float_as_uint(p_b);
            e[3] = __float_as_uint(factor);
            e[4] = __float_as_uint(ray.direction.x); e[5] = __float_as_uint(ray.direction.y);
            e[6] = __float_as_uint(ray.direction.z);
            npend += 1;
          }
          COLD(C_FIX) = ((uint32_t)(fix + 2) << 2) | (uint32_t)npend;
        }
        o += 1;
        ev = EV_START;
        ended = true;
      } else if (ev == EV_HIT || ev == EV_HIT_COLOR_PENDING) {
        i += 1;
        if (i > 10) {
          o += 1;
          ended = true;
        }
      } else if (ev == EV_NONE) {
        i += 1;
        if (i > 10) {
          o += 1;
          ev = EV_START;
          ended = true;
        }
      }

      if (ended && o > 2) {
        const int fix = (int)(COLD(C_FIX) >> 2) - 2;
        if (fix == -1)
          finish_item<MODE>(a, (int64_t)(((uint64_t)COLD_ENTRY_HI() << 32) | (uint64_t)COLD(C_ENTRY_LO)), COLD(C_HIT), COLD(C_PIXEL) & 0xFFFFu,
                            COLD(C_PIXEL) >> 16, COLD(C_BV_R), COLD(C_BV_G), COLD(C_BV_B));
        else if (fix >= 0) a.fixups[(size_t)fix * kFixupDwords + 7] = COLD(C_FIX) & 3u;
        st = ST_IDLE;
      } else {
        st = ST_EVENT + ev;
      }
    }

    const unsigned long long idle_mask = __ballot(st == ST_IDLE);
    const uint32_t n_idle = (uint32_t)__popcll(idle_mask);
    if (!exhausted && n_idle >= (uint32_t)a.refill_min_lanes) {
      const uint32_t NQ = (uint32_t)a.unit_queues, S = (uint32_t)a.n_seeds, G = (uint32_t)a.unit_group;
      const uint32_t KB = (uint32_t)a.unit_block_log2, n_blocks = (n_chunks + (1u << KB) - 1u) >> KB;
      uint32_t base = 0u, count = 0u, q_sel = 0u;
      if (lane == 0u) {
        for (uint32_t tries = 0; tries < NQ && count == 0u; ++tries) {
          const uint32_t q = (home_queue + tries) % NQ;
          const uint32_t blocks_q = (n_blocks + NQ - 1u - q) / NQ;
          const uint32_t chunks_q = blocks_q << KB;
          if (chunks_q == 0u || ((queue_dry >> q) & 1u)) continue;
          const uint32_t total = chunks_q * S * 64u;
          const uint32_t p = atomicAdd(&a.counters[CTR_QUEUE_STRIDE * (q + 1u)], n_idle);
          if (p + n_idle >= total) queue_dry |= 1u << q;
          if (p < total) {
            base = p;
            count = min(n_idle, total - p);
            q_sel = q;
          }
        }
      }
      base = __shfl(base, 0);
      count = __shfl(count, 0);
      q_sel = __shfl(q_sel, 0);
      stats.refill(count);
      if (count == 0u) {
        exhausted = true;
      } else if (st == ST_IDLE) {
        const uint32_t rank = (uint32_t)__popcll(idle_mask & ((1ull << lane) - 1ull));
        if (rank < count) {
          const uint32_t item = base + rank, p = item >> 6;
          const uint32_t chunks_q = ((n_blocks + NQ - 1u - q_sel) / NQ) << KB;
          uint32_t r, c_in;
          const uint32_t g = udivmod24(p, G * S, r);
          const uint32_t in_group = min(G, chunks_q - g * G);
          const uint32_t s = udivmod24(r, in_group, c_in), ch = g * G + c_in;
          const uint32_t chunk = ((q_sel + NQ * (ch >> KB)) << KB) + (ch & ((1u << KB) - 1u));
          const uint32_t h = chunk * 64u + (item & 63u);
          if (h < n_hits) {
            const uint4 *src = reinterpret_cast<const uint4 *>(&a.hits[h]);
            const uint4 q0 = src[0], q1 = src[1], q2 = src[2], q3 = src[3];
            const f3 hit_origin = f3{__uint_as_float(q0.x), __uint_as_float(q0.y), __uint_as_float(q0.z)};
            const f3 hit_direction = f3{__uint_as_float(q0.w), __uint_as_float(q1.x), __uint_as_float(q1.y)};
            const f3 start = hit_origin + hit_direction;
            color = q2.y;
            const int64_t entry = (int64_t)(((uint64_t)q2.w << 32) | (uint64_t)q2.z);
            bool granted = true;
            if (MODE == CLWH_ACCUM_VOXEL_CACHE)
              granted = a.grants ? s < a.grants[h] : (entry >= 0 && cache_take_token(a.cache, entry, 256u));
            if (granted) {
              COLD(C_START_X) = __float_as_uint(start.x); COLD(C_START_Y) = __float_as_uint(start.y); COLD(C_START_Z) = __float_as_uint(start.z);
              COLD(C_NORMAL_X) = q1.z; COLD(C_NORMAL_Y) = q1.w; COLD(C_NORMAL_Z) = q2.x;
              COLD(C_ENTRY_LO) = q2.z; COLD(C_ENTRY_HI) = (q2.w & 0xFFu) | (hull_cert ? (a.hull_codes[h] & 0x1FFFu) << 8 : 0u) | (q3.z << 24);
              COLD(C_PIXEL) = q3.x;
              COLD(C_HIT) = h;
              COLD(C_SEED) = (uint32_t)a.seeds[s];
              COLD(C_FIX) = (uint32_t)(-1 + 2) << 2;
              COLD(C_BV_R) = 0u; COLD(C_BV_G) = 0u; COLD(C_BV_B) = 0u;
              r_energy = div255[color & 255u];
              g_energy = div255[(color >> 8) & 255u];
              b_energy = div255[(color >> 16) & 255u];
              o = 1;
              st = ST_EVENT + EV_START;
            } else if (a.contrib_out) {
              uint32_t *q = a.contrib_out + ((size_t)(q3.x >> 16) * (size_t)a.launch_w + (q3.x & 0xFFFFu)) * 4;
              q[0] = 0u; q[1] = 0u; q[2] = 0u; q[3] = 0u;
            }
          }
        }
      }
    }
    stats.fresh_items(st, o);
    if (__ballot(st != ST_IDLE) == 0ull) {
      if (exhausted && lane == 0u) stats.flush<false>(a.counters);
      if (exhausted) break;
      continue;
    }

    bool sc_tried = false, sc_granted = false;
    bool hc_tried = false, hc_granted = false;
    if (st >= ST_EVENT) {
      const int ev = st - ST_EVENT;
      bool start_path = (ev == EV_START);
      bool bounce = false, from_hit = false;
      f3 bn{0, 0, 0}, bstart{0, 0, 0};
      int bseed = 0;

      if (ev == EV_HIT || ev == EV_HIT_COLOR_PENDING) {
        bn = -normalize3(hit_gradient_and_color<SMALL>(vol, a.tf, ray.origin, ev == EV_HIT_COLOR_PENDING, color));
        bstart = ray.origin + ray.direction;
        bseed = o + i - 1;
        bounce = true;
        from_hit = true;
        if (i > 10) {
          r_energy *= div255[color & 255u];
          g_energy *= div255[(color >> 8) & 255u];
          b_energy *= div255[(color >> 16) & 255u];
          bounce = false;
          start_path = true;
        }
      }

      if (start_path) {
        bn = f3{__uint_as_float(COLD(C_NORMAL_X)), __uint_as_float(COLD(C_NORMAL_Y)), __uint_as_float(COLD(C_NORMAL_Z))};
        bstart = f3{__uint_as_float(COLD(C_START_X)), __uint_as_float(COLD(C_START_Y)), __uint_as_float(COLD(C_START_Z))};
        bseed = o;
        bounce = true;
        from_hit = false;
      }

      if (bounce) {
        const float roughness = div255[color >> 24];
        const uint32_t pixel = COLD(C_PIXEL);
        Ray nr;
        nr.direction = hemisphere_reflective(pixel & 0xFFFFu, pixel >> 16, bn, (int)COLD(C_SEED) + bseed, roughness);
        nr.origin = bstart + bn * 2.0f;
        const float d = fabsf(dot3(nr.direction, bn));
        if (from_hit) {
          atten *= d;
          r_energy *= div255[color & 255u];
          g_energy *= div255[(color >> 8) & 255u];
          b_energy *= div255[(color >> 16) & 255u];
        } else {
          atten = d;
          i = 8;
          if (start_cert) {
            sc_tried = true;
            const uint32_t word = COLD(C_ENTRY_HI);
            sc_granted = start_certificate(word >> 24, nr.direction, a.start_cert_dmin);
            if (hull_cert) {
              hc_tried = (word & 0x001FFF00u) != 0u;
              hc_granted = hull_certificate((word >> 8) & 0x1FFFu, nr.direction, a.hull_delta0);
            }
          }
        }
        ray = nr;
      }

      if ((sc_granted || hc_granted) && !kStartCertVerify) {
        st = ST_EVENT + EV_EXIT;
      } else {
        sd = (int)(vol.template step_i<SMALL>(f2i(ray.origin.x), f2i(ray.origin.y), f2i(ray.origin.z)) & 0x7Fu);
        march = 70u * kOneStep + kCertReady;
        st = ST_MARCH;
      }
    }
    stats.start_cert(sc_tried, sc_granted);
    stats.hull_cert(hc_tried, hc_granted, hc_granted && sc_granted);
  }
#undef COLD_ENTRY_HI
#undef COLD
}

hipError_t launch_bounce(const RenderArgs &a_in, hipStream_t s) {
  RenderArgs a = a_in;
  const uint64_t total = (uint64_t)a.n_hits * (uint64_t)a.n_seeds;
  if (total == 0) return hipSuccess;
  const uint64_t waves_needed = (total + 63u) / 64u;
  constexpr unsigned wpb = (unsigned)kBounceThreads / 64u;
  const unsigned blocks = (unsigned)std::min<uint64_t>((waves_needed + wpb - 1u) / wpb, ((uint64_t)a.bounce_max_blocks * 4u + wpb - 1u) / wpb);
  const dim3 grid(blocks), block(kBounceThreads);
  const uint64_t waves_likely = ((uint64_t)a.n_hits_estimate * (uint64_t)a.n_seeds + 63u) / 64u;
  const bool long_launch = a.force_long_launch || waves_likely >= 6u * (uint64_t)blocks * wpb;
  if (a.step_min_lanes <= 0) a.step_min_lanes = long_launch ? 16 : 1;
  if (a.refill_min_lanes <= 0) a.refill_min_lanes = long_launch ? 16 : 64;
  a.cert_min_lanes = kCertPhaseMinLanes;
  if (!long_launch) a.cert_min_step = 0;
  if (!bounce_queues_fit(a.n_hits, a.unit_block_log2, a.n_seeds)) return hipErrorInvalidValue;
  const bool g = a.tf.uses_gradient != 0;
  const bool small = (uint64_t)a.NBX * (uint64_t)a.NBY * (uint64_t)((a.Z + 7) / 8) < (1ull << 23) &&
                     a.X + a.Y + a.Z <= VolumePacked::kPartsMaxEntries;
  const size_t lds_parts_bytes = small ? (size_t)(a.X + a.Y + a.Z) * sizeof(uint32_t) : 0u;
  const bool two_rays = a.bounce_rays == 2 && long_launch && a.n_hits < (1u << 26) && kBounceThreads == 256;
  if (two_rays) a.fixup_capacity = std::min<uint32_t>(a.fixup_capacity, (1u << 27) - 4u);
#define CLVR_LAUNCH_BOUNCE(G, M)                                                                    \
  do {                                                                                              \
    if (two_rays) {                                                                                 \
      if (small) hipLaunchKernelGGL((k_bounce2<G, M, true>), grid, block, lds_parts_bytes, s, a);  \
      else hipLaunchKernelGGL((k_bounce2<G, M, false>), grid, block, 0, s, a);                     \
    } else if (small) hipLaunchKernelGGL((k_bounce<G, M, true>), grid, block, lds_parts_bytes, s, a); \
    else hipLaunchKernelGGL((k_bounce<G, M, false>), grid, block, 0, s, a);                        \
  } while (0)
  if (a.mode == CLWH_ACCUM_VOXEL_CACHE) {
    if (g) CLVR_LAUNCH_BOUNCE(true, CLWH_ACCUM_VOXEL_CACHE);
    else CLVR_LAUNCH_BOUNCE(false, CLWH_ACCUM_VOXEL_CACHE);
  } else {
    if (g) CLVR_LAUNCH_BOUNCE(true, CLWH_ACCUM_IMAGE_SPACE);
    else CLVR_LAUNCH_BOUNCE(false, CLWH_ACCUM_IMAGE_SPACE);
  }
#undef CLVR_LAUNCH_BOUNCE
  return hipGetLastError();
}

}
```

cl_volume_renderer_amd/ffi.py:

```python
from __future__ import annotations

import ctypes as C
import os

import numpy as np

_HERE = os.path.dirname(os.path.abspath(__file__))
LIB_PATH = os.environ.get("CLWH_LIBRARY") or os.path.join(_HERE, "libclwhip.so")

OK = 0
ELEM_S8, ELEM_S16, ELEM_S32, ELEM_U8, ELEM_U16, ELEM_U32, ELEM_F32 = range(7)
ARG_MEM, ARG_I32, ARG_U32, ARG_F32, ARG_I64, ARG_U64, ARG_F64 = range(7)
ACCUM_VOXEL_CACHE, ACCUM_IMAGE_SPACE = 0, 1
DERIVED_SCENE, DERIVED_CAMERA, DERIVED_PROJECTION = 1, 2, 4
PROJ_MAX, PROJ_MIN, PROJ_MEAN = 0, 1, 2
PROJ_DENSE = 1
COMP_DENSE, COMP_SHADE = 1, 2
ISO_DENSE, ISO_BELOW = 1, 2
SLICE_MAX, SLICE_MIN, SLICE_MEAN = 0, 1, 2
SLICE_DENSE = 1
MESH_DENSE, MESH_BELOW = 1, 2
GROW_26, GROW_FROM_MASK, GROW_DENSE = 1, 2, 4
GROW_MAX_SEEDS = 65536
LABEL_26, LABEL_FROM_MASK = 1, 2
# ... 181 lines not shown
        ("volume", C.c_void_p), ("labels", C.c_void_p), ("components", C.c_void_p), ("component_capacity", C.c_uint64),
        ("mask", C.c_void_p),
        ("lo", C.c_int32), ("hi", C.c_int32), ("flags", C.c_int32),
        ("box_lo", C.c_uint32 * 3), ("box_hi", C.c_uint32 * 3),
        ("result", C.POINTER(LabelResult)),
    ]


class LabelsToMaskDesc(C.Structure):
    _fields_ = [("labels", C.c_void_p), ("mask", C.c_void_p), ("dims", C.c_uint32 * 3), ("rank_lo", C.c_uint32), ("rank_hi", C.c_uint32)]


class DistanceDesc(C.Structure):
    _fields_ = [("mask", C.c_void_p), ("dist", C.c_void_p), ("dims", C.c_uint32 * 3), ("weight", C.c_uint32 * 3), ("cap", C.c_uint32),
                ("flags", C.c_int32)]


class MorphDesc(C.Structure):
    _fields_ = [("mask_in", C.c_void_p), ("mask_out", C.c_void_p), ("dims", C.c_uint32 * 3), ("weight", C.c_uint32 * 3),
                ("radius_sq", C.c_uint32), ("op", C.c_int32), ("flags", C.c_int32)]


class MaskCombineDesc(C.Structure):
    _fields_ = [("a", C.c_void_p), ("b", C.c_void_p), ("out", C.c_void_p), ("dims", C.c_uint32 * 3), ("op", C.c_int32)]


class RegionStats(C.Structure):
    _fields_ = [
        ("count", C.c_uint64), ("sum", C.c_int64), ("sum_sq", C.c_uint64),
        ("vmin", C.c_int32), ("vmax", C.c_int32),
        ("sum_pos", C.c_uint64 * 3),
        ("bbox_lo", C.c_uint32 * 3), ("bbox_hi", C.c_uint32 * 3),
        ("faces", C.c_uint32 * 3), ("border_faces", C.c_uint32 * 3),
    ]

    def as_dict(self):
        return {"count": int(self.count), "sum": int(self.sum), "sum_sq": int(self.sum_sq), "vmin": int(self.vmin), "vmax": int(self.vmax),
                "sum_pos": tuple(int(v) for v in self.sum_pos), "bbox_lo": tuple(self.bbox_lo), "bbox_hi": tuple(self.bbox_hi),
                "faces": tuple(self.faces), "border_faces": tuple(self.border_faces)}


REGION_STATS_DTYPE = np.dtype([("count", np.uint64), ("sum", np.int64), ("sum_sq", np.uint64), ("vmin", np.int32), ("vmax", np.int32),
                               ("sum_pos", np.uint64, (3,)), ("bbox_lo", np.uint32, (3,)), ("bbox_hi", np.uint32, (3,)),
                               ("faces", np.uint32, (3,)), ("border_faces", np.uint32, (3,))])
assert REGION_STATS_DTYPE.itemsize == C.sizeof(RegionStats) == 104
LABEL_STATS_MAX_CAPACITY = 1 << 24


class MaskStatsResult(C.Structure):
    _fields_ = [("stats", RegionStats), ("hist_below", C.c_uint64), ("hist_above", C.c_uint64)]


class MaskStatsDesc(C.Structure):
    _fields_ = [("volume", C.c_void_p), ("mask", C.c_void_p), ("hist", C.c_void_p), ("hist_lo", C.c_int32), ("bin_width", C.c_int32),
                ("n_bins", C.c_int32), ("flags", C.c_int32), ("result", C.POINTER(MaskStatsResult))]


class LabelStatsDesc(C.Structure):
    _fields_ = [("volume", C.c_void_p), ("labels", C.c_void_p), ("stats", C.c_void_p), ("capacity", C.c_uint64), ("flags", C.c_int32),
                ("reserved", C.c_int32)]


class OverlayRegion(C.Structure):
    _fields_ = [("buffer", C.c_void_p), ("kind", C.c_int32), ("dims", C.c_uint32 * 3), ("id_lo", C.c_uint32), ("id_hi", C.c_uint32)]


class OverlayPaint(C.Structure):
    _fields_ = [("palette", C.c_void_p), ("n_colours", C.c_uint32), ("flags", C.c_int32), ("fill_alpha", C.c_uint32),
                ("outline_alpha", C.c_uint32), ("ids", C.c_void_p), ("t_first", C.c_void_p)]


class OverlaySliceDesc(C.Structure):
    _fields_ = [
        ("frame", C.c_void_p), ("region", OverlayRegion), ("paint", OverlayPaint),
        ("origin", C.c_float * 3), ("du", C.c_float * 3), ("dv", C.c_float * 3), ("normal", C.c_float * 3),
        ("width", C.c_uint32), ("height", C.c_uint32),
        ("slab_samples", C.c_int32), ("step", C.c_float),
    ]


class OverlayCameraDesc(C.Structure):
    _fields_ = [
        ("frame", C.c_void_p), ("region", OverlayRegion), ("paint", OverlayPaint),
        ("cam_pos", C.c_float * 3), ("cam_dir", C.c_float * 3),
        ("width", C.c_uint32), ("height", C.c_uint32),
        ("step", C.c_float), ("t_near", C.c_float), ("t_far", C.c_float), ("reserved", C.c_int32),
    ]


_SIZE3 = C.POINTER(C.c_size_t)
_PROTOTYPES = [
    ("clwh_ctx_create", C.c_int, [C.c_int, C.POINTER(C.c_void_p)]),
    ("clwh_ctx_create_on_stream", C.c_int, [C.c_int, C.c_void_p, C.POINTER(C.c_void_p)]),
    ("clwh_ctx_destroy", C.c_int, [C.c_void_p]),
    ("clwh_ctx_finish", C.c_int, [C.c_void_p]),
    ("clwh_ctx_stream", C.c_void_p, [C.c_void_p]),
    ("clwh_ctx_device", C.c_int, [C.c_void_p]),
    ("clwh_mem_create", C.c_int, [C.c_void_p, C.c_size_t, C.c_int, C.POINTER(C.c_void_p)]),
    ("clwh_mem_wrap", C.c_int, [C.c_void_p, C.c_void_p, C.c_size_t, C.POINTER(C.c_void_p)]),
    ("clwh_image_create", C.c_int, [C.c_void_p, _SIZE3, C.c_int, C.c_int, C.c_int, C.POINTER(C.c_void_p)]),
    ("clwh_image_wrap", C.c_int, [C.c_void_p, C.c_void_p, _SIZE3, C.c_int, C.c_int, C.POINTER(C.c_void_p)]),
    ("clwh_mem_push", C.c_int, [C.c_void_p, C.c_void_p, C.c_void_p, C.c_size_t]),
    ("clwh_mem_pull", C.c_int, [C.c_void_p, C.c_void_p, C.c_void_p, C.c_size_t]),
    ("clwh_mem_release", C.c_int, [C.c_void_p]),
    ("clwh_host_register", C.c_int, [C.c_void_p, C.c_size_t]),
    ("clwh_host_unregister", C.c_int, [C.c_void_p]),
    ("clwh_mem_device_ptr", C.c_void_p, [C.c_void_p]),
    ("clwh_mem_size", C.c_size_t, [C.c_void_p]),
    ("clwh_mem_mark_dirty", C.c_int, [C.c_void_p]),
    ("clwh_kernel_get", C.c_int, [C.c_void_p, C.c_char_p, C.c_char_p, C.c_char_p, C.POINTER(C.c_void_p)]),
    ("clwh_kernel_release", C.c_int, [C.c_void_p]),
    ("clwh_launch", C.c_int, [C.c_void_p, _SIZE3, _SIZE3, C.POINTER(Arg), C.c_int]),
    ("clwh_render", C.c_int, [C.c_void_p, C.POINTER(RenderDesc)]),
    ("clwh_cache_len", C.c_int64, [C.c_uint32, C.c_uint32, C.c_uint32]),
    ("clwh_accum_len", C.c_int64, [C.c_uint32, C.c_uint32, C.c_int32]),
    ("clwh_accum_resolve", C.c_int, [C.c_void_p, C.c_void_p, C.c_int32, C.c_uint32, C.c_uint32, C.c_void_p,
                                     C.c_void_p, C.POINTER(C.c_float), C.POINTER(C.c_float)]),
    ("clwh_accum_resolve_tiles", C.c_int, [C.c_void_p, C.c_void_p, C.c_int32, C.c_int32, C.c_uint32, C.c_uint32, C.c_void_p,
                                           C.c_void_p, C.POINTER(C.c_float), C.POINTER(C.c_float)]),
    ("clwh_frame_from_tiles", C.c_int, [C.c_void_p, C.c_void_p, C.c_int32, C.c_uint32, C.c_uint32, C.c_void_p]),
    ("clwh_ctx_invalidate_derived", C.c_int, [C.c_void_p, C.c_int]),
    ("clwh_ctx_scene_info", C.c_int, [C.c_void_p, C.POINTER(C.c_uint64), C.POINTER(C.c_uint64), C.POINTER(C.c_int32)]),
    ("clwh_render_projection", C.c_int, [C.c_void_p, C.POINTER(ProjectionDesc)]),
    ("clwh_render_composite", C.c_int, [C.c_void_p, C.POINTER(CompositeDesc)]),
    ("clwh_render_isosurface", C.c_int, [C.c_void_p, C.POINTER(IsosurfaceDesc)]),
    ("clwh_render_slice", C.c_int, [C.c_void_p, C.POINTER(SliceDesc)]),
    ("clwh_mesh_isosurface", C.c_int, [C.c_void_p, C.POINTER(MeshDesc)]),
    ("clwh_segment_grow", C.c_int, [C.c_void_p, C.POINTER(GrowDesc)]),
    ("clwh_volume_apply_mask", C.c_int, [C.c_void_p, C.POINTER(ApplyMaskDesc)]),
    ("clwh_segment_label", C.c_int, [C.c_void_p, C.POINTER(LabelDesc)]),
    ("clwh_labels_to_mask", C.c_int, [C.c_void_p, C.POINTER(LabelsToMaskDesc)]),
    ("clwh_mask_distance", C.c_int, [C.c_void_p, C.POINTER(DistanceDesc)]),
    ("clwh_mask_morph", C.c_int, [C.c_void_p, C.POINTER(MorphDesc)]),
    ("clwh_mask_combine", C.c_int, [C.c_void_p, C.POINTER(MaskCombineDesc)]),
    ("clwh_mask_statistics", C.c_int, [C.c_void_p, C.POINTER(MaskStatsDesc)]),
    ("clwh_label_statistics", C.c_int, [C.c_void_p, C.POINTER(LabelStatsDesc)]),
    ("clwh_overlay_slice", C.c_int, [C.c_void_p, C.POINTER(OverlaySliceDesc)]),
    ("clwh_overlay_camera", C.c_int, [C.c_void_p, C.POINTER(OverlayCameraDesc)]),
    ("clwh_sdf_build", C.c_int, [C.c_void_p, C.c_void_p, C.c_char_p, C.c_void_p, C.POINTER(C.c_int32)]),
    ("clwh_buffer_reset", C.c_int, [C.c_void_p, C.c_void_p]),
    ("clwh_cache_exchange_plan", C.c_int, [C.c_void_p, C.c_void_p, C.c_uint64, C.POINTER(C.c_void_p)]),
    ("clwh_cache_apply_contributions", C.c_int, [C.c_void_p, C.c_void_p, C.c_void_p, C.c_void_p, C.c_int32]),
    ("clwh_cache_exchange_plan_release", C.c_int, [C.c_void_p]),
    ("clwh_tf_parse", C.c_int, [C.c_char_p, C.POINTER(Tf)]),
    ("clwh_debug_float_conversions", C.c_int, [C.c_void_p, C.c_void_p, C.c_uint64, C.c_void_p, C.c_void_p]),
    ("clwh_debug_wave_min", C.c_int, [C.c_void_p, C.c_void_p, C.c_uint64, C.c_void_p]),
    ("clwh_debug_macro_table", C.c_int, [C.c_void_p, C.c_void_p, C.c_uint64, C.POINTER(C.c_int32)]),
    ("clwh_debug_start_table", C.c_int, [C.c_void_p, C.c_void_p, C.c_uint64, C.POINTER(C.c_int32)]),
    ("clwh_debug_start_cert_dmin", C.c_int, [C.c_int32, C.c_int32, C.c_int32, C.POINTER(C.c_float)]),
    ("clwh_debug_hit_records", C.c_int, [C.c_void_p, C.c_void_p, C.c_uint64, C.POINTER(C.c_uint32)]),
    ("clwh_debug_hull_table", C.c_int, [C.c_void_p, C.c_void_p, C.c_uint64, C.POINTER(C.c_int32)]),
    ("clwh_debug_hull_cert_bound", C.c_int, [C.c_int32, C.c_int32, C.c_int32, C.POINTER(C.c_float)]),
    ("clwh_debug_hull_codes", C.c_int, [C.c_void_p, C.c_void_p, C.c_uint64, C.POINTER(C.c_uint32)]),
    ("clwh_strerror", C.c_char_p, [C.c_int]),
    ("clwh_last_hip_error", C.c_int, []),
    ("clwh_version", C.c_char_p, []),
    ("clwh_ctx_acquire_from", C.c_int, [C.c_void_p, C.c_void_p]),
    ("clwh_ctx_release_to", C.c_int, [C.c_void_p, C.c_void_p]),
    ("clwh_ctx_set_timing", C.c_int, [C.c_void_p, C.c_int]),
    ("clwh_ctx_timing_read", C.c_int, [C.c_void_p, C.POINTER(C.c_float), C.POINTER(C.c_int32)]),
    ("clwh_ctx_timing_read_all", C.c_int, [C.c_void_p, C.POINTER(C.c_float), C.POINTER(C.c_int32), C.c_int32]),
]
EXPORTED_SYMBOLS = [p[0] for p in _PROTOTYPES]

_lib = None


def lib():
    global _lib
    if _lib is None:
        if not os.path.exists(LIB_PATH):
            raise RuntimeError(
                "libclwhip.so is missing (%s): build it with `python -m cl_volume_renderer_amd.build`; "
                "there is no CPU fallback for the product path" % LIB_PATH)
        L = C.CDLL(LIB_PATH)
        for name, res, args in _PROTOTYPES:
            if not hasattr(L, name) and os.environ.get("CLWH_LIBRARY"):
                continue
            f = getattr(L, name)
            f.restype = res
            f.argtypes = args
        _lib = L
    return _lib


def _check(status, where):
    if status != OK:
        raise ClwhError(status, where)


def parse_tf(source: str) -> Tf:
    tf = Tf()
    _check(lib().clwh_tf_parse(source.encode(), C.byref(tf)), "clwh_tf_parse")
    return tf


def hull_cert_bound(X: int, Y: int, Z: int):
    v = (C.c_float * 2)()
    _check(lib().clwh_debug_hull_cert_bound(X, Y, Z, v), "clwh_debug_hull_cert_bound")
    return float(v[0]), float(v[1])


def start_cert_dmin(X: int, Y: int, Z: int) -> float:
    v = C.c_float(0)
    _check(lib().clwh_debug_start_cert_dmin(X, Y, Z, C.byref(v)), "clwh_debug_start_cert_dmin")
    return float(v.value)


def cache_len(X, Y, Z) -> int:
    return int(lib().clwh_cache_len(X, Y, Z))


def accum_len(w, h, world=1) -> int:
    return int(lib().clwh_accum_len(w, h, world))


def _handle(mem):
    return mem.h if mem is not None else None


def _fill_overlay(d, frame, source, kind, dims, palette, width, height, n_colours, flags, fill_alpha, outline_alpha, id_range, ids, t_first):
    d.frame = _handle(frame)
    d.region.buffer, d.region.kind = _handle(source), int(kind)
    for k in range(3):
        d.region.dims[k] = int(dims[k])
    d.region.id_lo, d.region.id_hi = int(id_range[0]), int(id_range[1])
    d.paint.palette = _handle(palette)
    d.paint.n_colours = int(n_colours if n_colours is not None else (palette.nbytes // 4 if palette is not None else 0))
    d.paint.flags, d.paint.fill_alpha, d.paint.outline_alpha = int(flags), int(fill_alpha), int(outline_alpha)
    d.paint.ids, d.paint.t_first = _handle(ids), _handle(t_first)
    d.width, d.height = int(width), int(height)


def _fill_view(d, frame, volume, cam_pos, cam_dir, width, height):
    d.frame, d.volume = frame.h, volume.h
    for k in range(3):
        d.cam_pos[k] = float(cam_pos[k])
        d.cam_dir[k] = float(cam_dir[k])
    d.width, d.height = int(width), int(height)


class Mem:
    def __init__(self, ctx, handle, nbytes, dtype=None, shape=None):
        self.ctx, self.h, self.nbytes, self.dtype, self.shape = ctx, C.c_void_p(handle), nbytes, dtype, shape

    def push(self, arr: np.ndarray):
        a = np.ascontiguousarray(arr)
        _check(lib().clwh_mem_push(self.ctx.h, self.h, a.ctypes.data, a.nbytes), "clwh_mem_push")

    def pull(self, dtype=None, shape=None) -> np.ndarray:
        dtype = np.dtype(dtype or self.dtype or np.uint8)
        out = np.empty(self.nbytes // dtype.itemsize, dtype=dtype)
        _check(lib().clwh_mem_pull(self.ctx.h, self.h, out.ctypes.data, out.nbytes), "clwh_mem_pull")
        shape = shape or self.shape
        return out.reshape(shape) if shape else out

    @property
    def device_ptr(self) -> int:
        return int(lib().clwh_mem_device_ptr(self.h) or 0)

    def release(self):
        if self.h:
            _check(lib().clwh_mem_release(self.h), "clwh_mem_release")
            self.h = None


class Kernel:
    def __init__(self, ctx, handle):
        self.ctx, self.h = ctx, C.c_void_p(handle)

    def launch(self, global_size, local_size, *args):
        g = (C.c_size_t * 3)(*(list(global_size) + [0, 0, 0])[:3])
        l = (C.c_size_t * 3)(*(list(local_size) + [0, 0, 0])[:3])
        arr = (Arg * max(len(args), 1))()
        for i, a in enumerate(args):
            if isinstance(a, Mem):
                arr[i].kind, arr[i].v.mem = ARG_MEM, a.h.value
            elif isinstance(a, (float, np.floating)):
                arr[i].kind, arr[i].v.f32 = ARG_F32, float(a)
            elif isinstance(a, np.unsignedinteger):
                arr[i].kind, arr[i].v.u32 = ARG_U32, int(a)
            elif isinstance(a, (int, np.integer)):
                arr[i].kind, arr[i].v.i32 = ARG_I32, int(a)
            else:
                raise TypeError("unsupported kernel argument %r" % (a,))
        _check(lib().clwh_launch(self.h, g, l, arr, len(args)), "clwh_launch")

    def render(self, *, frame, volume, sdf, env, cam_pos, cam_dir, seed, width, height, buffer_volume=None,
               accum=None, mode=ACCUM_VOXEL_CACHE, tile_rank=0, tile_world=1, write_frame=True,
               hit_index=None, contrib=None, seeds=None, shading=SHADE_LIGHT, resolve_only=False):
        d = RenderDesc()
        d.frame = frame.h if frame is not None else None
        d.volume, d.sdf, d.env = volume.h, sdf.h, env.h
        d.buffer_volume = buffer_volume.h if buffer_volume is not None else None
        for k in range(3):
            d.cam_pos[k] = float(cam_pos[k])
            d.cam_dir[k] = float(cam_dir[k])
        d.seed, d.width, d.height = int(seed), int(width), int(height)
        d.accum_mode = mode
        d.accum = accum.h if accum is not None else None
        d.tile_rank, d.tile_world = tile_rank, tile_world
        d.write_frame = 1 if write_frame else 0
        d.hit_index = hit_index.h if hit_index is not None else None
        d.contrib = contrib.h if contrib is not None else None
        d.shading = shading
        d.resolve_only = 1 if resolve_only else 0
        if seeds is not None:
            d.n_seeds = len(seeds)
            for i, sd in enumerate(seeds):
                d.seeds[i] = int(sd)
        _check(lib().clwh_render(self.h, C.byref(d)), "clwh_render")

    def release(self):
        if self.h:
            _check(lib().clwh_kernel_release(self.h), "clwh_kernel_release")
            self.h = None


class ExchangePlan:
    def __init__(self, ctx, handle):
        self.ctx, self.h = ctx, C.c_void_p(handle)

    def apply(self, buffer_volume: Mem, rgb: Mem, rgb_stride=3):
        _check(lib().clwh_cache_apply_contributions(self.ctx.h, self.h, buffer_volume.h, rgb.h, rgb_stride),
               "clwh_cache_apply_contributions")

    def release(self):
        if self.h:
            _check(lib().clwh_cache_exchange_plan_release(self.h), "clwh_cache_exchange_plan_release")
            self.h = None


class Context:
    def __init__(self, device=0, stream=None):
        h = C.c_void_p()
        if stream is None:
            _check(lib().clwh_ctx_create(device, C.byref(h)), "clwh_ctx_create")
        else:
            _check(lib().clwh_ctx_create_on_stream(device, C.c_void_p(stream), C.byref(h)),
                   "clwh_ctx_create_on_stream")
        self.h = h

    def buffer(self, nbytes, dtype=None, shape=None) -> Mem:
        h = C.c_void_p()
        _check(lib().clwh_mem_create(self.h, nbytes, 0, C.byref(h)), "clwh_mem_create")
        return Mem(self, h.value, nbytes, dtype, shape)

    def buffer_from(self, arr: np.ndarray) -> Mem:
        a = np.ascontiguousarray(arr)
        m = self.buffer(a.nbytes, a.dtype, a.shape)
        m.push(a)
        return m

# ... 284 lines not shown
            if largest is not None:
                if int(largest) < 1:
                    raise ValueError("largest is at least 1")
                keep = min(n, int(largest))
            else:
                keep = int(np.count_nonzero(table["count"] >= int(min_count)))
                if keep == len(table) and len(table) < n:
                    raise ValueError("min_count=%d is not decided by the %d largest of %d components: pass a larger capacity"
                                     % (int(min_count), len(table), n))
            dims = volume.shape[::-1]
            out = self.labels_to_mask(labels, dims, 1 if keep else n + 1, keep if keep else n + 1)
            return out, res, keep
        finally:
            labels.release()

    def mask_distance_raw(self, mask: Mem, dist: Mem, dims, weights=(1, 1, 1), cap=DIST_NONE, flags=0):
        d = DistanceDesc()
        d.mask, d.dist = _handle(mask), _handle(dist)
        for k in range(3):
            d.dims[k], d.weight[k] = int(dims[k]), int(weights[k])
        d.cap, d.flags = int(cap), int(flags)
        return lib().clwh_mask_distance(self.h, C.byref(d))

    def mask_distance(self, mask: Mem, dims, weights=(1, 1, 1), to_clear=False, cap=None, dist: Mem = None) -> Mem:
        own = dist is None
        if own:
            shape = (int(dims[2]), int(dims[1]), int(dims[0]))
            dist = self.buffer(4 * int(np.prod(shape)), np.uint32, shape)
        status = self.mask_distance_raw(mask, dist, dims, weights, DIST_NONE if cap is None else cap, DIST_TO_CLEAR if to_clear else 0)
        if status != OK and own:
            dist.release()
        _check(status, "clwh_mask_distance")
        return dist

    def _new_mask(self, dims) -> Mem:
        from . import scene

        n = scene.mask_words_per_row(int(dims[0])) * int(dims[1]) * int(dims[2])
        return self.buffer(4 * n, np.uint32, (n,))

    def mask_morph_raw(self, mask_in: Mem, mask_out: Mem, dims, op, radius_sq, weights=(1, 1, 1), flags=0):
        d = MorphDesc()
        d.mask_in, d.mask_out = _handle(mask_in), _handle(mask_out)
        for k in range(3):
            d.dims[k], d.weight[k] = int(dims[k]), int(weights[k])
        d.radius_sq, d.op, d.flags = int(radius_sq), int(op), int(flags)
        return lib().clwh_mask_morph(self.h, C.byref(d))

    def mask_morph(self, mask: Mem, dims, op, radius_sq, weights=(1, 1, 1), out: Mem = None) -> Mem:
        own = out is None
        if own:
            out = self._new_mask(dims)
        status = self.mask_morph_raw(mask, out, dims, op, radius_sq, weights)
        if status != OK and own:
            out.release()
        _check(status, "clwh_mask_morph")
        return out

    def mask_combine_raw(self, a: Mem, b: Mem, out: Mem, dims, op):
        d = MaskCombineDesc()
        d.a, d.b, d.out = _handle(a), _handle(b), _handle(out)
        for k in range(3):
            d.dims[k] = int(dims[k])
        d.op = int(op)
        return lib().clwh_mask_combine(self.h, C.byref(d))

    def mask_combine(self, a: Mem, b: Mem, op, dims, out: Mem = None) -> Mem:
        own = out is None
        if own:
            out = self._new_mask(dims)
        status = self.mask_combine_raw(a, b, out, dims, op)
        if status != OK and own:
            out.release()
        _check(status, "clwh_mask_combine")
        return out

    def mask_statistics_raw(self, volume: Mem, mask: Mem, hist: Mem = None, hist_lo=0, bin_width=0, n_bins=0, flags=0, result=True):
        d, res = MaskStatsDesc(), MaskStatsResult()
        d.volume, d.mask, d.hist = _handle(volume), _handle(mask), _handle(hist)
        d.hist_lo, d.bin_width, d.n_bins, d.flags = int(hist_lo), int(bin_width), int(n_bins), int(flags)
        if result:
            d.result = C.pointer(res)
        return lib().clwh_mask_statistics(self.h, C.byref(d)), res

    def mask_statistics(self, volume: Mem, mask: Mem, hist=None):
        table = None
        try:
            if hist is not None:
                lo, width, n = (int(v) for v in hist)
                table = self.buffer(8 * max(n, 1), np.uint64, (max(n, 1),))
                status, res = self.mask_statistics_raw(volume, mask, table, lo, width, n)
            else:
                status, res = self.mask_statistics_raw(volume, mask)
            _check(status, "clwh_mask_statistics")
            counts = table.pull()[:int(hist[2])].copy() if table is not None else None
            return res.stats, counts, int(res.hist_below), int(res.hist_above)
        finally:
            if table is not None:
                table.release()

    def label_statistics_raw(self, volume: Mem, labels: Mem, stats: Mem, capacity, flags=0):
        d = LabelStatsDesc()
        d.volume, d.labels, d.stats = _handle(volume), _handle(labels), _handle(stats)
        d.capacity, d.flags = int(capacity), int(flags)
        return lib().clwh_label_statistics(self.h, C.byref(d))

    def label_statistics(self, volume: Mem, labels: Mem, capacity, stats: Mem = None) -> Mem:
        own = stats is None
        if own:
            stats = self.buffer(104 * max(int(capacity), 1), REGION_STATS_DTYPE, (max(int(capacity), 1),))
        status = self.label_statistics_raw(volume, labels, stats, capacity)
        if status != OK and own:
            stats.release()
        _check(status, "clwh_label_statistics")
        return stats

    def scene_info(self):
        sid, nb, holders = C.c_uint64(0), C.c_uint64(0), C.c_int32(0)
        _check(lib().clwh_ctx_scene_info(self.h, C.byref(sid), C.byref(nb), C.byref(holders)), "clwh_ctx_scene_info")
        return int(sid.value), int(nb.value), int(holders.value)

    def macro_table(self):
        info = (C.c_int32 * 4)()
        _check(lib().clwh_debug_macro_table(self.h, None, C.c_uint64(0), info), "clwh_debug_macro_table")
        out = np.empty((info[2], info[1], info[0], 8), np.uint8)
        _check(lib().clwh_debug_macro_table(self.h, out.ctypes.data_as(C.c_void_p), C.c_uint64(out.nbytes), info), "clwh_debug_macro_table")
        return out, int(info[3])

    def start_table(self):
        info = (C.c_int32 * 4)()
        _check(lib().clwh_debug_start_table(self.h, None, C.c_uint64(0), info), "clwh_debug_start_table")
        if not info[3]:
            return None
        out = np.empty((info[2], info[1], info[0]), np.uint8)
        _check(lib().clwh_debug_start_table(self.h, out.ctypes.data_as(C.c_void_p), C.c_uint64(out.nbytes), info), "clwh_debug_start_table")
        return out

    def hull_table(self):
        info = (C.c_int32 * 4)()
        _check(lib().clwh_debug_hull_table(self.h, None, C.c_uint64(0), info), "clwh_debug_hull_table")
        if not info[3]:
            return None
        out = np.empty((info[1], 4), np.float32)
        _check(lib().clwh_debug_hull_table(self.h, out.ctypes.data_as(C.c_void_p), C.c_uint64(out.nbytes), info), "clwh_debug_hull_table")
        return out

    def hull_codes(self):
        n = C.c_uint32(0)
        _check(lib().clwh_debug_hull_codes(self.h, None, C.c_uint64(0), C.byref(n)), "clwh_debug_hull_codes")
        out = np.empty(int(n.value), np.uint32)
        _check(lib().clwh_debug_hull_codes(self.h, out.ctypes.data_as(C.c_void_p), C.c_uint64(out.nbytes), C.byref(n)), "clwh_debug_hull_codes")
        return out[:int(n.value)]

    def hit_records(self):
        n = C.c_uint32(0)
        _check(lib().clwh_debug_hit_records(self.h, None, C.c_uint64(0), C.byref(n)), "clwh_debug_hit_records")
        out = np.empty((int(n.value), 16), np.uint32)
        _check(lib().clwh_debug_hit_records(self.h, out.ctypes.data_as(C.c_void_p), C.c_uint64(out.nbytes), C.byref(n)), "clwh_debug_hit_records")
        return out[:int(n.value)]

    def image_wrap(self, device_ptr: int, dims, channels, dtype, shape=None) -> Mem:
        dtype = np.dtype(dtype)
        d = (C.c_size_t * 3)(*(list(dims) + [1, 1, 1])[:3])
        h = C.c_void_p()
        _check(lib().clwh_image_wrap(self.h, C.c_void_p(device_ptr), d, channels, _ELEM_OF_DTYPE[dtype], C.byref(h)),
               "clwh_image_wrap")
        n = int(np.prod([max(int(x), 1) for x in list(dims)[:3]])) * channels * dtype.itemsize
        return Mem(self, h.value, n, dtype, shape)

    def acquire_from(self, stream: int):
        _check(lib().clwh_ctx_acquire_from(self.h, C.c_void_p(stream)), "clwh_ctx_acquire_from")

    def release_to(self, stream: int):
        _check(lib().clwh_ctx_release_to(self.h, C.c_void_p(stream)), "clwh_ctx_release_to")

    def finish(self):
        _check(lib().clwh_ctx_finish(self.h), "clwh_ctx_finish")

    def set_timing(self, enabled=True):
        _check(lib().clwh_ctx_set_timing(self.h, 1 if enabled else 0), "clwh_ctx_set_timing")

    def timing_read(self):
        ms, n = C.c_float(0), C.c_int32(0)
        _check(lib().clwh_ctx_timing_read(self.h, C.byref(ms), C.byref(n)), "clwh_ctx_timing_read")
        return float(ms.value), int(n.value)

    def timing_read_all(self):
        n = len(TIMERS)
        ms, cnt = (C.c_float * n)(), (C.c_int32 * n)()
        _check(lib().clwh_ctx_timing_read_all(self.h, ms, cnt, n), "clwh_ctx_timing_read_all")
        return {name: (float(ms[i]), int(cnt[i])) for i, name in enumerate(TIMERS)}

    @property
    def stream(self) -> int:
        return int(lib().clwh_ctx_stream(self.h) or 0)

    def destroy(self):
        if self.h:
            _check(lib().clwh_ctx_destroy(self.h), "clwh_ctx_destroy")
            self.h = None
```

include/clwh.h:

```cpp
#ifndef CLWH_H
#define CLWH_H

#include <stddef.h>
#include <stdint.h>

#ifdef __cplusplus
extern "C" {
#endif

typedef struct clwh_ctx clwh_ctx;
typedef struct clwh_mem clwh_mem;
typedef struct clwh_kernel clwh_kernel;

enum clwh_status {
  CLWH_OK = 0,
  CLWH_ERR_INVALID_VALUE = 1,
  CLWH_ERR_NO_DEVICE = 2,
  CLWH_ERR_OUT_OF_MEMORY = 3,
  CLWH_ERR_HIP = 4,
  CLWH_ERR_UNKNOWN_KERNEL = 5,
  CLWH_ERR_TF_UNSUPPORTED = 6,
  CLWH_ERR_BAD_ARGS = 7,
  CLWH_ERR_BAD_NDRANGE = 8,
  CLWH_ERR_SIZE_MISMATCH = 9,
// ... 266 lines not shown
int clwh_labels_to_mask(clwh_ctx *ctx, const clwh_labels_to_mask_desc *desc);

#define CLWH_DIST_NONE 0xFFFFFFFFu
enum clwh_distance_flags { CLWH_DIST_TO_CLEAR = 1 };
typedef struct clwh_distance_desc {
  clwh_mem *mask;
  clwh_mem *dist;
  uint32_t dims[3];
  uint32_t weight[3];
  uint32_t cap;
  int32_t flags;
} clwh_distance_desc;
int clwh_mask_distance(clwh_ctx *ctx, const clwh_distance_desc *desc);

enum clwh_morph_op { CLWH_MORPH_DILATE = 0, CLWH_MORPH_ERODE = 1, CLWH_MORPH_OPEN = 2, CLWH_MORPH_CLOSE = 3 };
typedef struct clwh_morph_desc {
  clwh_mem *mask_in;
  clwh_mem *mask_out;
  uint32_t dims[3];
  uint32_t weight[3];
  uint32_t radius_sq;
  int32_t op;
  int32_t flags;
} clwh_morph_desc;
int clwh_mask_morph(clwh_ctx *ctx, const clwh_morph_desc *desc);

enum clwh_mask_op { CLWH_MASK_AND = 0, CLWH_MASK_OR = 1, CLWH_MASK_XOR = 2, CLWH_MASK_ANDNOT = 3, CLWH_MASK_NOT = 4 };
typedef struct clwh_mask_combine_desc {
  clwh_mem *a;
  clwh_mem *b;
  clwh_mem *out;
  uint32_t dims[3];
  int32_t op;
} clwh_mask_combine_desc;
int clwh_mask_combine(clwh_ctx *ctx, const clwh_mask_combine_desc *desc);

typedef struct clwh_region_stats {
  uint64_t count;
  int64_t sum;
  uint64_t sum_sq;
  int32_t vmin, vmax;
  uint64_t sum_pos[3];
  uint32_t bbox_lo[3], bbox_hi[3];
  uint32_t faces[3];
  uint32_t border_faces[3];
} clwh_region_stats;

typedef struct clwh_mask_stats_result {
  clwh_region_stats stats;
  uint64_t hist_below, hist_above;
} clwh_mask_stats_result;
typedef struct clwh_mask_stats_desc {
  clwh_mem *volume;
  clwh_mem *mask;
  clwh_mem *hist;
  int32_t hist_lo;
  int32_t bin_width;
  int32_t n_bins;
  int32_t flags;
  clwh_mask_stats_result *result;
} clwh_mask_stats_desc;
int clwh_mask_statistics(clwh_ctx *ctx, const clwh_mask_stats_desc *desc);

typedef struct clwh_label_stats_desc {
  clwh_mem *volume;
  clwh_mem *labels;
  clwh_mem *stats;
  uint64_t capacity;
  int32_t flags;
  int32_t reserved;
} clwh_label_stats_desc;
int clwh_label_statistics(clwh_ctx *ctx, const clwh_label_stats_desc *desc);

enum clwh_region_kind { CLWH_REGION_MASK = 0, CLWH_REGION_LABELS = 1 };
enum clwh_overlay_flags {
  CLWH_OVERLAY_FILL = 1,
  CLWH_OVERLAY_OUTLINE = 2,
  CLWH_OVERLAY_DENSE = 4
};
typedef struct clwh_overlay_region {
  clwh_mem *buffer;
  int32_t kind;
  uint32_t dims[3];
  uint32_t id_lo, id_hi;
} clwh_overlay_region;
typedef struct clwh_overlay_paint {
  clwh_mem *palette;
  uint32_t n_colours;
  int32_t flags;
  uint32_t fill_alpha, outline_alpha;
  clwh_mem *ids;
  clwh_mem *t_first;
} clwh_overlay_paint;
typedef struct clwh_overlay_slice_desc {
  clwh_mem *frame;
  clwh_overlay_region region;
  clwh_overlay_paint paint;
  float origin[3], du[3], dv[3], normal[3];
  uint32_t width, height;
  int32_t slab_samples;
  float step;
} clwh_overlay_slice_desc;
typedef struct clwh_overlay_camera_desc {
  clwh_mem *frame;
  clwh_overlay_region region;
  clwh_overlay_paint paint;
  float cam_pos[3], cam_dir[3];
  uint32_t width, height;
  float step;
  float t_near, t_far;
  int32_t reserved;
} clwh_overlay_camera_desc;
int clwh_overlay_slice(clwh_ctx *ctx, const clwh_overlay_slice_desc *desc);
int clwh_overlay_camera(clwh_ctx *ctx, const clwh_overlay_camera_desc *desc);

int clwh_sdf_build(clwh_ctx *ctx, clwh_mem *volume, const char *tf_source, clwh_mem *sdf,
                   int32_t *n_launches);

int clwh_buffer_reset(clwh_ctx *ctx, clwh_mem *buffer_volume);

typedef struct clwh_exchange_plan clwh_exchange_plan;
int clwh_cache_exchange_plan(clwh_ctx *ctx, clwh_mem *entries, uint64_t n, clwh_exchange_plan **out);
int clwh_cache_apply_contributions(clwh_ctx *ctx, clwh_exchange_plan *plan, clwh_mem *buffer_volume, clwh_mem *rgb,
                                   int32_t rgb_stride);
int clwh_cache_exchange_plan_release(clwh_exchange_plan *plan);

int clwh_ctx_acquire_from(clwh_ctx *ctx, void *hip_stream);
int clwh_ctx_release_to(clwh_ctx *ctx, void *hip_stream);

#define CLWH_TF_MAX_RULES 16
typedef struct clwh_tf_rule {
  int32_t v_lo, v_hi;
  int32_t g_lo, g_hi;
  int32_t use_gradient;
  int32_t writes_color;
  int32_t terminal;
  int32_t color[4];
} clwh_tf_rule;
typedef struct clwh_tf {
  int32_t n;
  clwh_tf_rule rules[CLWH_TF_MAX_RULES];
} clwh_tf;
int clwh_tf_parse(const char *source, clwh_tf *out);

int clwh_debug_float_conversions(clwh_ctx *ctx, clwh_mem *floats_in, uint64_t n, clwh_mem *i32_out, clwh_mem *u32_out);
int clwh_debug_wave_min(clwh_ctx *ctx, clwh_mem *u32_in, uint64_t n, clwh_mem *u32_out);
int clwh_debug_macro_table(clwh_ctx *ctx, void *host_out, uint64_t capacity, int32_t info_out[4]);
int clwh_debug_start_table(clwh_ctx *ctx, void *host_out, uint64_t capacity, int32_t info_out[4]);
int clwh_debug_start_cert_dmin(int32_t X, int32_t Y, int32_t Z, float *dmin_out);
int clwh_debug_hit_records(clwh_ctx *ctx, void *host_out, uint64_t capacity, uint32_t *n_hits_out);
int clwh_debug_hull_table(clwh_ctx *ctx, void *host_out, uint64_t capacity, int32_t info_out[4]);
int clwh_debug_hull_cert_bound(int32_t X, int32_t Y, int32_t Z, float out[2]);
int clwh_debug_hull_codes(clwh_ctx *ctx, void *host_out, uint64_t capacity, uint32_t *n_hits_out);
const char *clwh_strerror(int status);
int clwh_last_hip_error(void);
const char *clwh_version(void);
int clwh_ctx_set_timing(clwh_ctx *ctx, int enabled);
int clwh_ctx_timing_read(clwh_ctx *ctx, float *total_ms, int32_t *launches);
enum clwh_timer {
  CLWH_TIMER_BOUNCE = 0,
  CLWH_TIMER_PRIMARY = 1,
  CLWH_TIMER_FIXUP = 2,
  CLWH_TIMER_RESOLVE = 3,
  CLWH_TIMER_REPACK = 4,
  CLWH_TIMER_AO = 5,
  CLWH_TIMER_COUNT = 6
};
int clwh_ctx_timing_read_all(clwh_ctx *ctx, float *ms, int32_t *launches, int32_t n);

#ifdef __cplusplus
}
#endif
#endif
```

Baseline: 44420.

## Add deferred hull exit certificates and hull checks for rebound rays

Stores a signed hull-plane margin per primary hit. Rays that start slightly behind the plane are armed to get a cheap exit certificate after a computed number of march steps, instead of running the full certify_exit test. The hull certificate is also applied to rebound rays that start from hit points, using the plane offset. This is meant to cut march steps and certification work per bounce. The cost is an extra per-hit buffer, repacking of the cold entry word into fewer bits, and more branch logic in the bounce kernel.

```diff
diff --git a/cl_volume_renderer_amd/csrc/bounce_device.hpp b/cl_volume_renderer_amd/csrc/bounce_device.hpp
--- a/cl_volume_renderer_amd/csrc/bounce_device.hpp
+++ b/cl_volume_renderer_amd/csrc/bounce_device.hpp
@@ -76,12 +76,6 @@
   const float x = z >= 0.0f ? u : copysignf(1.0f - fabsf(v), u), y = z >= 0.0f ? v : copysignf(1.0f - fabsf(u), v);
   const float r = __builtin_amdgcn_rsqf((x * x + y * y) + z * z);
   return f3{x * r, y * r, z * r};
-}
-__device__ __forceinline__ bool hull_certificate(uint32_t code, f3 d, float delta0) {
-  const f3 n = hull_direction(code - 1u);
-  const float dmin = fminf(fminf(fabsf(d.x), fabsf(d.y)), fabsf(d.z));
-  const float dsum = d.x + d.y + d.z;
-  return code != 0u && dot3(d, n) >= delta0 && dmin >= 0.0009765625f && dsum == dsum;
 }
 __device__ __forceinline__ bool certify_exit(const RenderArgs &a, f3 p, f3 d, int budget) {
   int away;
@@ -125,6 +119,8 @@
   __device__ void swap_point() {}
   __device__ void start_cert(bool, bool) {}
   __device__ void hull_cert(bool, bool, bool) {}
+  __device__ void hull_more(bool, bool, bool, bool) {}
+  __device__ void hull_fired(bool, bool) {}
   __device__ void march_end(uint32_t *, int) {}
   template <bool TWO_RAYS> __device__ void flush(uint32_t *) {}
 };
@@ -174,11 +170,24 @@
     hull_both += (uint32_t)__popcll(__ballot(both));
     hull_open = hull_open || granted;
   }
+  uint32_t more_tried[3] = {0, 0, 0}, more_granted[3] = {0, 0, 0};
+  int more_open = -1;
+  __device__ __forceinline__ void hull_more(bool rebound_tried, bool rebound_granted, bool armed, bool first_leg) {
+    more_tried[0] += (uint32_t)__popcll(__ballot(armed && first_leg)); more_tried[2] += (uint32_t)__popcll(__ballot(armed && !first_leg));
+    more_tried[1] += (uint32_t)__popcll(__ballot(rebound_tried)); more_granted[1] += (uint32_t)__popcll(__ballot(rebound_granted));
+    if (rebound_granted) more_open = 1;
+  }
+  __device__ __forceinline__ void hull_fired(bool fired, bool first_leg) {
+    more_granted[0] += (uint32_t)__popcll(__ballot(fired && first_leg)); more_granted[2] += (uint32_t)__popcll(__ballot(fired && !first_leg));
+    if (fired) more_open = first_leg ? 0 : 2;
+  }
   __device__ __forceinline__ void march_end(uint32_t *counters, int ev) {
     if (start_open && ev != EV_EXIT) atomicAdd(&counters[CTR_START_WRONG], 1u);
     if (hull_open && ev != EV_EXIT) atomicAdd(&counters[CTR_HULL_WRONG], 1u);
+    if (more_open >= 0 && ev != EV_EXIT) atomicAdd(&counters[CTR_HULL_DEFER + 3 * more_open + 2], 1u);
     start_open = false;
     hull_open = false;
+    more_open = -1;
   }
   template <bool TWO_RAYS> __device__ __forceinline__ void flush(uint32_t *counters) {
     atomicAdd(&counters[CTR_STEP_ITERS], step_iters); atomicAdd(&counters[CTR_STEP_LANES], step_lanes);
@@ -190,6 +199,7 @@
     atomicAdd(&counters[CTR_CERT_GRANTED], cert_granted); atomicAdd(&counters[CTR_STEP_IDLE], step_idle);
     atomicAdd(&counters[CTR_START_TRIED], start_tried); atomicAdd(&counters[CTR_START_GRANTED], start_granted);
     atomicAdd(&counters[CTR_HULL_TRIED], hull_tried); atomicAdd(&counters[CTR_HULL_GRANTED], hull_granted); atomicAdd(&counters[CTR_HULL_BOTH], hull_both);
+    for (int k = 0; k < 3; ++k) { atomicAdd(&counters[CTR_HULL_DEFER + 3 * k], more_tried[k]); atomicAdd(&counters[CTR_HULL_DEFER + 3 * k + 1], more_granted[k]); }
   }
 };
 using BounceStats = BounceStatsT<kBounceStats>;
diff --git a/cl_volume_renderer_amd/csrc/clwh_context.hip b/cl_volume_renderer_amd/csrc/clwh_context.hip
--- a/cl_volume_renderer_amd/csrc/clwh_context.hip
+++ b/cl_volume_renderer_amd/csrc/clwh_context.hip
@@ -155,6 +155,7 @@
   if (const char *e = std::getenv("CLWH_TUNE_CERT_HINT")) t.cert_hint = std::atoi(e) != 0;
   if (const char *e = std::getenv("CLWH_TUNE_START_CERT")) t.start_cert = std::atoi(e) != 0;
   if (const char *e = std::getenv("CLWH_TUNE_HULL_CERT")) t.hull_cert = std::atoi(e) != 0;
+  if (const char *e = std::getenv("CLWH_TUNE_HULL_DEFER")) t.hull_defer = std::atoi(e) != 0;
   return t;
 }
 
diff --git a/cl_volume_renderer_amd/csrc/clwh_host.hpp b/cl_volume_renderer_amd/csrc/clwh_host.hpp
--- a/cl_volume_renderer_amd/csrc/clwh_host.hpp
+++ b/cl_volume_renderer_amd/csrc/clwh_host.hpp
@@ -119,6 +119,7 @@
   int32_t cert_hint = 1;
   int32_t start_cert = 1;
   int32_t hull_cert = 1;
+  int32_t hull_defer = 1;
   int32_t cert_min_step = -1;
   uint32_t bounce_max_blocks = 2048;
   int32_t sdfbit_waves = 8;
@@ -145,6 +146,7 @@
   bool valid = false;
   DeviceBuffer pix_slot, hits;
   DeviceBuffer hull_codes;
+  DeviceBuffer hull_planes;
   uint32_t n_hits = 0;
   bool n_hits_known = false;
   PinnedWord host_n_hits;
@@ -154,7 +156,7 @@
 };
 
 struct PassScratch {
-  static constexpr size_t kCounters = CTR_QUEUE_STRIDE * 9;
+  static constexpr size_t kCounters = CTR_QUEUE_STRIDE * 10;
   DeviceBuffer counters;
   DeviceBuffer fixups, delta;
   DeviceBuffer sticky_flags;
diff --git a/cl_volume_renderer_amd/csrc/clwh_internal.hpp b/cl_volume_renderer_amd/csrc/clwh_internal.hpp
--- a/cl_volume_renderer_amd/csrc/clwh_internal.hpp
+++ b/cl_volume_renderer_amd/csrc/clwh_internal.hpp
@@ -52,6 +52,7 @@
   CTR_HULL_TRIED, CTR_HULL_GRANTED, CTR_HULL_BOTH, CTR_HULL_WRONG,
   CTR_STATS_END,
   CTR_QUEUE_STRIDE = 32,
+  CTR_HULL_DEFER = CTR_QUEUE_STRIDE * 9, CTR_HULL_DEFER_END = CTR_HULL_DEFER + 9,
 };
 struct RenderArgs {
   int32_t X, Y, Z;
@@ -69,6 +70,8 @@
   const float4 *hull;
   uint32_t *hull_codes;
   float hull_delta0;
+  uint32_t *hull_planes;
+  float hull_defer_delta0;
   int32_t NBX, NBY;
   const uint32_t *env;
   int32_t env_w, env_h;
@@ -189,6 +192,24 @@
   }
   return 2.0f;
 }
+constexpr int kHullDeferSteps = 3;
+constexpr float kHullDeferDeficit = 1.5f;
+constexpr int kHullMarginScale = 16;
+inline float hull_defer_delta0(int X, int Y, int Z) {
+  const double longest = (double)(X > Y ? (X > Z ? X : Z) : (Y > Z ? Y : Z));
+  const double reach = 1.7320508075688772 * (longest + 1.0), cap = (double)start_cert_cap(X, Y, Z);
+  for (int k = 1; k <= 64; ++k) {
+    const double delta0 = (double)k / 64.0;
+    double t = 0.0;
+    for (int step = 0; step < 70 - 5 - kHullDeferSteps && t <= reach; ++step) {
+      const double m = (double)(long long)(t * delta0 / 1.7320508075688772) - 2.0;
+      const double bound = m > cap ? cap : m;
+      t += bound < 1.0 ? 1.0 : bound;
+    }
+    if (t > reach) return (float)delta0;
+  }
+  return 2.0f;
+}
 hipError_t launch_hull_table(const int2 *ends, const uint32_t *regular, float4 *hull, int X, int Y, int Z, hipStream_t s);
 constexpr uint64_t kStartTableBudget = 2ull << 30;
 hipError_t launch_primary(const RenderArgs &a, hipStream_t s);
diff --git a/cl_volume_renderer_amd/csrc/clwh_render.hip b/cl_volume_renderer_amd/csrc/clwh_render.hip
--- a/cl_volume_renderer_amd/csrc/clwh_render.hip
+++ b/cl_volume_renderer_amd/csrc/clwh_render.hip
@@ -236,6 +236,7 @@
   a.cert_hint = t.cert_hint;
   a.start_cert_dmin = start_cert_dmin(a.X, a.Y, a.Z);
   a.hull_delta0 = hull_cert_delta0(a.X, a.Y, a.Z);
+  a.hull_defer_delta0 = hull_defer_delta0(a.X, a.Y, a.Z);
   return CLWH_OK;
 }
 
@@ -273,6 +274,8 @@
   CLWH_TRY(p.pix_slot.reserve(ctx->stream, slots * sizeof(uint32_t)));
   CLWH_TRY(p.hits.reserve(ctx->stream, slots * sizeof(HitRec)));
   if (a.hull) CLWH_TRY(p.hull_codes.reserve(ctx->stream, slots * sizeof(uint32_t)));
+  const bool defer = a.hull && ctx->tune.hull_defer != 0;
+  if (defer) CLWH_TRY(p.hull_planes.reserve(ctx->stream, slots * sizeof(uint32_t)));
   CLWH_TRY(s.counters.reserve(ctx->stream, PassScratch::kCounters * sizeof(uint32_t)));
   bool fresh_flags = false;
   CLWH_TRY(s.sticky_flags.reserve(ctx->stream, 64, &fresh_flags));
@@ -281,6 +284,7 @@
   a.pix_slot = p.pix_slot.as<uint32_t>();
   a.hits = p.hits.as<HitRec>();
   a.hull_codes = a.hull ? p.hull_codes.as<uint32_t>() : nullptr;
+  a.hull_planes = defer ? p.hull_planes.as<uint32_t>() : nullptr;
   a.counters = s.counters.as<uint32_t>();
 
   PrimaryHits::Key key;
@@ -381,7 +385,7 @@
 
 #ifdef CLVR_BOUNCE_STATS
 static int print_bounce_stats(clwh_ctx *ctx, const RenderArgs &a) {
-  uint32_t h[CTR_STATS_END];
+  uint32_t h[CTR_HULL_DEFER_END];
   HIP_TRY(hipMemcpyAsync(h, a.counters, sizeof h, hipMemcpyDeviceToHost, ctx->stream));
   HIP_TRY(hipStreamSynchronize(ctx->stream));
   auto per = [&](int sum, int n) { return h[n] ? (double)h[sum] / h[n] : 0.0; };
@@ -398,6 +402,10 @@
   std::fprintf(stderr, "[bounce stats] hull certificates tried/granted/wrong=%u/%u/%u, of the granted the octant proof grants %u; either proof grants %u first legs; delta0=%.6f\n",
                h[CTR_HULL_TRIED], h[CTR_HULL_GRANTED], h[CTR_HULL_WRONG], h[CTR_HULL_BOTH], h[CTR_START_GRANTED] + h[CTR_HULL_GRANTED] - h[CTR_HULL_BOTH],
                (double)a.hull_delta0);
+  const uint32_t *m = h + CTR_HULL_DEFER;
+  std::fprintf(stderr, "[bounce stats] hull certificates tried/granted/wrong: first legs deferred=%u/%u/%u rebounds at once=%u/%u/%u rebounds deferred=%u/%u/%u; "
+               "J=%d D=%.4g defer_delta0=%.6f; look-ups=%u\n", m[0], m[1], m[2], m[3], m[4], m[5], m[6], m[7], m[8], kHullDeferSteps, (double)kHullDeferDeficit,
+               (double)a.hull_defer_delta0, h[CTR_CERT_LANES] - ((CLVR_BOUNCE_STATS + 0) == 2 ? m[1] + m[7] : 0u));
   return CLWH_OK;
 }
 #endif
@@ -601,6 +609,32 @@
   return CLWH_OK;
 }
 
+int clwh_debug_hull_defer_bound(int32_t X, int32_t Y, int32_t Z, float out[4]) {
+  if (!out || X < 1 || Y < 1 || Z < 1) return CLWH_ERR_INVALID_VALUE;
+  out[0] = hull_defer_delta0(X, Y, Z);
+  out[1] = (float)kHullDeferSteps;
+  out[2] = kHullDeferDeficit;
+  out[3] = (float)kHullMarginScale;
+  return CLWH_OK;
+}
+
+int clwh_debug_hull_planes(clwh_ctx *ctx, void *host_out, uint64_t capacity, uint32_t *n_hits_out) {
+  if (!ctx || !n_hits_out) return CLWH_ERR_INVALID_VALUE;
+  PrimaryHits &p = ctx->primary;
+  if (!p.valid || !p.hits.ptr || !ctx->pass.counters.ptr) return CLWH_ERR_BAD_ARGS;
+  HIP_TRY(hipSetDevice(ctx->device));
+  HIP_TRY(hipMemcpyAsync(n_hits_out, ctx->pass.counters.as<uint32_t>() + CTR_HITS, sizeof(uint32_t), hipMemcpyDeviceToHost, ctx->stream));
+  HIP_TRY(hipStreamSynchronize(ctx->stream));
+  if (!host_out) return CLWH_OK;
+  const bool built = ctx->scene && ctx->scene->hull_table && ctx->tune.hull_defer != 0 && p.hull_planes.ptr;
+  const size_t bytes = (size_t)*n_hits_out * sizeof(uint32_t);
+  if (capacity < bytes || (built && p.hull_planes.bytes < bytes)) return CLWH_ERR_SIZE_MISMATCH;
+  if (!built) { std::memset(host_out, 0, bytes); return CLWH_OK;}
+  HIP_TRY(hipMemcpyAsync(host_out, p.hull_planes.ptr, bytes, hipMemcpyDeviceToHost, ctx->stream));
+  HIP_TRY(hipStreamSynchronize(ctx->stream));
+  return CLWH_OK;
+}
+
 int clwh_debug_hull_codes(clwh_ctx *ctx, void *host_out, uint64_t capacity, uint32_t *n_hits_out) {
   if (!ctx || !n_hits_out) return CLWH_ERR_INVALID_VALUE;
   PrimaryHits &p = ctx->primary;
diff --git a/cl_volume_renderer_amd/csrc/primary_kernels.hip b/cl_volume_renderer_amd/csrc/primary_kernels.hip
--- a/cl_volume_renderer_amd/csrc/primary_kernels.hip
+++ b/cl_volume_renderer_amd/csrc/primary_kernels.hip
@@ -96,6 +96,14 @@
         }
       if (margin >= 0.0f) code = ((uint32_t)(bj * kHullGrid + bi) + 1u) | ((uint32_t)fminf(floorf(margin * 256.0f), 65535.0f) << 16);
       a.hull_codes[h] = code;
+      if (a.hull_planes) {
+        uint32_t word = 0u;
+        if (margin >= -kHullDeferDeficit) {
+          const int q = (int)fminf(floorf(margin * (float)kHullMarginScale), 127.0f);
+          word = ((uint32_t)(bj * kHullGrid + bi) + 1u) | (((uint32_t)q & 0xFFu) << 16);
+        }
+        a.hull_planes[h] = word;
+      }
     }
     q3.x = x | (y << 16); q3.y = pslot; q3.z = start_free; q3.w = 0u;
     uint4 *dst = reinterpret_cast<uint4 *>(&a.hits[h]);
diff --git a/cl_volume_renderer_amd/csrc/render_kernels.hip b/cl_volume_renderer_amd/csrc/render_kernels.hip
--- a/cl_volume_renderer_amd/csrc/render_kernels.hip
+++ b/cl_volume_renderer_amd/csrc/render_kernels.hip
@@ -38,7 +38,7 @@
                C_BV_R, C_BV_G, C_BV_B, C_FIELDS };
   __shared__ uint32_t cold[C_FIELDS][kBounceThreads];
 #define COLD(f) cold[f][threadIdx.x]
-#define COLD_ENTRY_HI() ((uint32_t)((int32_t)(COLD(C_ENTRY_HI) << 24) >> 24))
+#define COLD_ENTRY_HI() ((uint32_t)((int32_t)(COLD(C_ENTRY_HI) << (32 - entry_hi_bits)) >> (32 - entry_hi_bits)))
   Ray ray{{0, 0, 0}, {0, 0, 0}};
   float atten = 0.0f, r_energy = 0.0f, g_energy = 0.0f, b_energy = 0.0f;
   uint32_t color = 0u;
@@ -46,12 +46,15 @@
   int st = ST_IDLE;
   int sd = 0;
   uint32_t march = 0u;
-  constexpr uint32_t kOneStep = 1u << 24, kCertReady = 1u << 23;
+  constexpr uint32_t kOneStep = 1u << 24, kCertReady = 1u << 23, kArmed = 1u << 31;
   const bool cert_hint = a.cert_hint != 0;
   const int cert_min_lanes = a.cert_min_lanes;
   const int cert_at = a.cert_min_step != 0 ? a.cert_min_step : kCertNever;
   const bool start_cert = !USE_GRAD && a.cert_min_step != 0;
   const bool hull_cert = start_cert && a.hull_codes != nullptr;
+  const bool hull_defer = hull_cert && a.hull_planes != nullptr;
+  const int entry_hi_bits = hull_defer ? 3 : 8;
+  const uint32_t *hull_words = hull_defer ? a.hull_planes : a.hull_codes;
   bool exhausted = false;
   BounceStats stats;
 
@@ -70,8 +73,8 @@
               const unsigned q = vol.template step_marched<SMALL>(ray.origin.x, ray.origin.y, ray.origin.z);
               sd = (int)(q & 0x7Fu);
               if (q & 0x80u) st = ST_EVENT + EV_HIT_COLOR_PENDING;
-              else if (march < kOneStep) st = ST_EVENT + EV_NONE;
-              else if (sd >= cert_at && (march & kCertReady)) st = ST_CERT;
+              else if ((march & ~kArmed) < kOneStep) st = ST_EVENT + EV_NONE;
+              else if (((march & kArmed) | (uint32_t)sd) >= (uint32_t)cert_at && (march & kCertReady)) st = ST_CERT;
             } else {
               st = ST_EVENT + EV_CHECK;
             }
@@ -94,9 +97,14 @@
         const int n_cert = __popcll(__ballot(st == ST_CERT));
         if (n_cert != 0 && (n_cert >= cert_min_lanes || __popcll(__ballot(st == ST_MARCH)) < a.step_min_lanes)) {
           stats.cert_begin(st, n_cert);
+          const bool fired = !USE_GRAD && st == ST_CERT && (march & kArmed) != 0u && (march & ~kArmed) >= (uint32_t)(70 - kHullDeferSteps) * kOneStep;
+          stats.hull_fired(fired, i == 8);
           if (st == ST_CERT) {
+            if (!USE_GRAD) march &= ~kArmed;
             int away;
-            if (certify_exit(a, ray.origin, ray.direction, (int)(march >> 24), away)) {
+            if (fired && !kStartCertVerify) {
+              st = ST_EVENT + EV_EXIT;
+            } else if (certify_exit(a, ray.origin, ray.direction, (int)(march >> 24), away)) {
               st = ST_EVENT + EV_EXIT;
             } else {
               march = (march & ~(kOneStep - 1u)) | (kCertReady - (uint32_t)(cert_hint ? away : 0));
@@ -120,7 +128,7 @@
             ev = pending ? EV_HIT_COLOR_PENDING : EV_HIT;
             break;
           }
-          if (march < kOneStep) { ev = EV_NONE; break; }
+          if ((march & ~kArmed) < kOneStep) { ev = EV_NONE; break; }
           ray.origin = ray.origin + ray.direction * fmaxf((float)next_sd, 0.5f);
           march -= kOneStep;
         }
@@ -248,7 +256,9 @@
             if (granted) {
               COLD(C_START_X) = __float_as_uint(start.x); COLD(C_START_Y) = __float_as_uint(start.y); COLD(C_START_Z) = __float_as_uint(start.z);
               COLD(C_NORMAL_X) = q1.z; COLD(C_NORMAL_Y) = q1.w; COLD(C_NORMAL_Z) = q2.x;
-              COLD(C_ENTRY_LO) = q2.z; COLD(C_ENTRY_HI) = (q2.w & 0xFFu) | (hull_cert ? (a.hull_codes[h] & 0x1FFFu) << 8 : 0u) | (q3.z << 24);
+              COLD(C_ENTRY_LO) = q2.z;
+              const uint32_t plane = hull_cert ? hull_words[h] : 0u;
+              COLD(C_ENTRY_HI) = (q2.w & ((1u << entry_hi_bits) - 1u)) | ((plane & 0x1FFFu) << entry_hi_bits) | (plane & (hull_defer ? 0x00FF0000u : 0u)) | (q3.z << 24);
               COLD(C_PIXEL) = q3.x;
               COLD(C_HIT) = h;
               COLD(C_SEED) = (uint32_t)a.seeds[s];
@@ -276,6 +286,8 @@
 
     bool sc_tried = false, sc_granted = false;
     bool hc_tried = false, hc_granted = false;
+    bool rb_tried = false, rb_granted = false;
+    uint32_t armed_path = 0u;
     if (st >= ST_EVENT) {
       const int ev = st - ST_EVENT;
       bool start_path = (ev == EV_START);
@@ -325,25 +337,42 @@
             sc_tried = true;
             const uint32_t word = COLD(C_ENTRY_HI);
             sc_granted = start_certificate(word >> 24, nr.direction, a.start_cert_dmin);
-            if (hull_cert) {
-              hc_tried = (word & 0x001FFF00u) != 0u;
-              hc_granted = hull_certificate((word >> 8) & 0x1FFFu, nr.direction, a.hull_delta0);
-            }
-          }
+          }
+        }
+        if (hull_cert && (hull_defer || !from_hit)) {
+          const uint32_t word = COLD(C_ENTRY_HI);
+          const uint32_t code = (word >> entry_hi_bits) & 0x1FFFu;
+          const f3 n = hull_direction(code - 1u);
+          const float dn = dot3(nr.direction, n);
+          const f3 dir = nr.direction;
+          const bool dir_ok = fminf(fminf(fabsf(dir.x), fabsf(dir.y)), fabsf(dir.z)) >= 0.0009765625f && (dir.x + dir.y) + dir.z == (dir.x + dir.y) + dir.z;
+          float m = hull_defer ? (float)((int32_t)(word << 8) >> 24) * (1.0f / (float)kHullMarginScale) : 0.0f;
+          if (from_hit) {
+            const f3 p = f3{__uint_as_float(COLD(C_START_X)), __uint_as_float(COLD(C_START_Y)), __uint_as_float(COLD(C_START_Z))} +
+                         f3{__uint_as_float(COLD(C_NORMAL_X)), __uint_as_float(COLD(C_NORMAL_Y)), __uint_as_float(COLD(C_NORMAL_Z))} * 2.0f;
+            m = m + dot3(n, f3{nr.origin.x - p.x, nr.origin.y - p.y, nr.origin.z - p.z});
+          }
+          const bool tried = code != 0u, granted = tried && dir_ok && m >= 0.0f && dn >= a.hull_delta0;
+          if (from_hit) { rb_tried = tried; rb_granted = granted; }
+          else { hc_tried = tried && m >= 0.0f; hc_granted = granted; }
+          if (tried && dir_ok && !sc_granted && m < 0.0f && m >= -kHullDeferDeficit && dn >= a.hull_defer_delta0)
+            armed_path = (uint32_t)ceilf(-m * __builtin_amdgcn_rcpf(dn) * (1.0f + 0x1p-19f));
         }
         ray = nr;
       }
 
-      if ((sc_granted || hc_granted) && !kStartCertVerify) {
+      if ((sc_granted || hc_granted || rb_granted) && !kStartCertVerify) {
         st = ST_EVENT + EV_EXIT;
       } else {
         sd = (int)(vol.template step_i<SMALL>(f2i(ray.origin.x), f2i(ray.origin.y), f2i(ray.origin.z)) & 0x7Fu);
         march = 70u * kOneStep + kCertReady;
+        if (armed_path != 0u) march = kArmed + 70u * kOneStep + kCertReady - armed_path;
         st = ST_MARCH;
       }
     }
     stats.start_cert(sc_tried, sc_granted);
     stats.hull_cert(hc_tried, hc_granted, hc_granted && sc_granted);
+    stats.hull_more(rb_tried, rb_granted, armed_path != 0u && st == ST_MARCH, i == 8);
   }
 #undef COLD_ENTRY_HI
 #undef COLD
diff --git a/cl_volume_renderer_amd/ffi.py b/cl_volume_renderer_amd/ffi.py
--- a/cl_volume_renderer_amd/ffi.py
+++ b/cl_volume_renderer_amd/ffi.py
@@ -357,6 +357,8 @@
     ("clwh_debug_hull_table", C.c_int, [C.c_void_p, C.c_void_p, C.c_uint64, C.POINTER(C.c_int32)]),
     ("clwh_debug_hull_cert_bound", C.c_int, [C.c_int32, C.c_int32, C.c_int32, C.POINTER(C.c_float)]),
     ("clwh_debug_hull_codes", C.c_int, [C.c_void_p, C.c_void_p, C.c_uint64, C.POINTER(C.c_uint32)]),
+    ("clwh_debug_hull_planes", C.c_int, [C.c_void_p, C.c_void_p, C.c_uint64, C.POINTER(C.c_uint32)]),
+    ("clwh_debug_hull_defer_bound", C.c_int, [C.c_int32, C.c_int32, C.c_int32, C.POINTER(C.c_float)]),
     ("clwh_strerror", C.c_char_p, [C.c_int]),
     ("clwh_last_hip_error", C.c_int, []),
     ("clwh_version", C.c_char_p, []),
@@ -404,6 +406,12 @@
     v = (C.c_float * 2)()
     _check(lib().clwh_debug_hull_cert_bound(X, Y, Z, v), "clwh_debug_hull_cert_bound")
     return float(v[0]), float(v[1])
+
+
+def hull_defer_bound(X: int, Y: int, Z: int):
+    v = (C.c_float * 4)()
+    _check(lib().clwh_debug_hull_defer_bound(X, Y, Z, v), "clwh_debug_hull_defer_bound")
+    return float(v[0]), int(v[1]), float(v[2]), int(v[3])
 
 
 def start_cert_dmin(X: int, Y: int, Z: int) -> float:
@@ -994,6 +1002,13 @@
         _check(lib().clwh_debug_hull_codes(self.h, out.ctypes.data_as(C.c_void_p), C.c_uint64(out.nbytes), C.byref(n)), "clwh_debug_hull_codes")
         return out[:int(n.value)]
 
+    def hull_planes(self):
+        n = C.c_uint32(0)
+        _check(lib().clwh_debug_hull_planes(self.h, None, C.c_uint64(0), C.byref(n)), "clwh_debug_hull_planes")
+        out = np.empty(int(n.value), np.uint32)
+        _check(lib().clwh_debug_hull_planes(self.h, out.ctypes.data_as(C.c_void_p), C.c_uint64(out.nbytes), C.byref(n)), "clwh_debug_hull_planes")
+        return out[:int(n.value)]
+
     def hit_records(self):
         n = C.c_uint32(0)
         _check(lib().clwh_debug_hit_records(self.h, None, C.c_uint64(0), C.byref(n)), "clwh_debug_hit_records")
diff --git a/include/clwh.h b/include/clwh.h
--- a/include/clwh.h
+++ b/include/clwh.h
@@ -442,6 +442,8 @@
 int clwh_debug_hull_table(clwh_ctx *ctx, void *host_out, uint64_t capacity, int32_t info_out[4]);
 int clwh_debug_hull_cert_bound(int32_t X, int32_t Y, int32_t Z, float out[2]);
 int clwh_debug_hull_codes(clwh_ctx *ctx, void *host_out, uint64_t capacity, uint32_t *n_hits_out);
+int clwh_debug_hull_planes(clwh_ctx *ctx, void *host_out, uint64_t capacity, uint32_t *n_hits_out);
+int clwh_debug_hull_defer_bound(int32_t X, int32_t Y, int32_t Z, float out[4]);
 const char *clwh_strerror(int status);
 int clwh_last_hip_error(void);
 const char *clwh_version(void);
```

Result: faster. 46870, median of 6 (+5.5%).
